# jepsen-io/maelstrom

Measured on NVIDIA H100. Metric: simulated msgs/sec (broadcast, 4096 nodes), higher is better.
Workload: dtype int64

## Files before the change

include/maelstrom_b200.h:

```cpp
#ifndef MAELSTROM_B200_H
#define MAELSTROM_B200_H

#include <stddef.h>
#include <stdint.h>

#ifdef __cplusplus
extern "C" {
#endif

#define MS_ABI_VERSION 2


typedef struct ms_msg {
  uint64_t id;
  int64_t  deadline_ns;
  uint32_t src, dest;
  uint32_t msg_id;
  uint32_t in_reply_to;
  uint16_t type;
  uint16_t flags;
  uint32_t p0;
  uint64_t p1;
} ms_msg;

// ... 141 lines not shown

typedef struct ms_kv_gen_config {
  uint32_t n_clients;
  uint32_t value_range;
  uint32_t keys_per_group;
  int64_t  interval_ns;
  int64_t  timeout_ns;
  int64_t  time_limit_ns;
  int64_t  key_period_ns;
} ms_kv_gen_config;
enum { MS_HF_KV_READ = 2, MS_HF_KV_WRITE = 3, MS_HF_KV_CAS = 4 };
int ms_add_kv_clients(ms_sim* sim, const ms_kv_gen_config* cfg, uint32_t first_name);

int ms_schedule_ops(ms_sim* sim, const ms_op* ops, size_t n);

int      ms_step(ms_sim* sim, uint64_t n_rounds);
int      ms_run(ms_sim* sim, int64_t until_virtual_ns);
int64_t  ms_now(ms_sim* sim);
uint64_t ms_round(ms_sim* sim);
int      ms_set_idle_jump(ms_sim* sim, int enable);

int ms_net_drop(ms_sim* sim, uint32_t src, uint32_t dest);
int ms_net_heal(ms_sim* sim);
int ms_net_slow(ms_sim* sim);
int ms_net_fast(ms_sim* sim);
int ms_net_flaky(ms_sim* sim);
int ms_net_set_loss(ms_sim* sim, double p);
int ms_net_partition(ms_sim* sim, const uint32_t* component_id, size_t n);

typedef struct ms_nemesis_config {
  uint32_t group;
  uint32_t targets;
  int64_t  interval_ns;
  int64_t  start_ns;
  int64_t  time_limit_ns;
} ms_nemesis_config;
#define MS_H_NEMESIS 0xFFFFFFFFu
enum { MS_HF_NEM_ONE = 5, MS_HF_NEM_MAJORITY = 6, MS_HF_NEM_MINORITY_THIRD = 7, MS_HF_NEM_STOP = 8,
       MS_HF_NEM_MAJORITIES_RING = 9 };
int ms_set_nemesis(ms_sim* sim, const ms_nemesis_config* cfg);
int ms_nemesis_grudge(uint32_t seed_lo, uint32_t seed_hi, uint32_t cluster, uint32_t g, uint32_t op, uint32_t target,
                      uint32_t* side_out);

int ms_journal_open(ms_sim* sim, const char* path);
int ms_journal_close(ms_sim* sim);
int ms_journal_drain(ms_sim* sim, ms_event* events, ms_jbody* bodies, size_t cap, size_t* n_out);
uint64_t ms_journal_written(ms_sim* sim);

enum { MS_JFMT_EVENT = 32, MS_JFMT_12 = 12, MS_JFMT_8 = 8, MS_JFMT_4 = 4,
       MS_JFMT_16 = 16 };
typedef struct ms_jround {
  uint64_t round;
  int64_t  time_ns;
  uint64_t ev_base;
  uint64_t id_ref;
} ms_jround;
typedef struct ms_jbatch {
  uint64_t first_event, n_events;
  uint64_t n_rounds;
  int64_t  now;
  uint64_t round, next_event;
  uint32_t format, overflow, more, error;
  uint64_t range_events;
} ms_jbatch;
typedef int (*ms_journal_sink)(void* ctx, const ms_jbatch* batch, const ms_jround* rounds, const void* events);
int ms_run_streamed(ms_sim* sim, int64_t until_virtual_ns, int format, size_t buf_events,
                    ms_journal_sink sink, void* ctx);
int ms_journal_decode(const ms_jbatch* batch, const ms_jround* rounds, const void* events, ms_event* out);
typedef struct ms_jdecoder ms_jdecoder;
ms_jdecoder* ms_jdecoder_create(uint32_t log2_window);
void ms_jdecoder_destroy(ms_jdecoder* dec);
int ms_jdecoder_decode(ms_jdecoder* dec, const ms_jbatch* batch, const ms_jround* rounds, const void* events, ms_event* out);
int ms_jdecoder_note(ms_jdecoder* dec, const ms_event* events, size_t n);
const char* ms_jdecoder_error(const ms_jdecoder* dec);

int ms_stats(ms_sim* sim, uint64_t out[9]);

size_t   ms_node_set(ms_sim* sim, uint32_t node, uint32_t* values, size_t cap);
uint64_t ms_client_replies(ms_sim* sim);
uint64_t ms_undeliverable(ms_sim* sim);
int      ms_raft_state(ms_sim* sim, uint32_t node, uint64_t out[8]);

int ms_counters(ms_sim* sim, uint64_t out[8]);

int ms_ring_counters(ms_sim* sim, uint64_t* out, uint32_t n);

int ms_set_origin(ms_sim* sim, uint64_t round, uint64_t msg_id, uint64_t event_id, uint32_t ring_pos,
                  uint32_t ring_stride);

#define MS_SHARD_BLOB_BYTES 512
typedef void (*ms_barrier_fn)(void* ctx, void* cuda_stream);
int   ms_shard_handles(ms_sim* sim, void* blob_out);
int   ms_shard_connect(ms_sim* sim, uint32_t peer, const void* blob);
int   ms_set_barrier(ms_sim* sim, ms_barrier_fn fn, void* ctx);
void* ms_stream(ms_sim* sim);
uint32_t ms_shard_owner(uint32_t e, uint32_t n_servers, uint32_t n_shards);

int ms_timer_begin(ms_sim* sim);
int ms_timer_end(ms_sim* sim, double* elapsed_ms);
int ms_profile(ms_sim* sim, int enable);
int ms_profile_read(ms_sim* sim, double* round_kernel_ms, uint64_t* launches);
int ms_debug_phase_cycles(ms_sim* sim, int enable, uint64_t out[64]);

size_t ms_topology(uint32_t topology, uint32_t n, uint32_t node, uint32_t* out, size_t cap);

#ifdef __cplusplus
}
#endif
#endif
```

integration/java/maelstrom/b200/Native.java:

```java
package maelstrom.b200;

import java.nio.ByteBuffer;

public final class Native {
  static { System.loadLibrary("ms_jni"); }
  private Native() {}

  public interface JournalSink { int accept(ByteBuffer batch, ByteBuffer rounds, ByteBuffer events); }

  public static native int abiVersion();
  public static native long create(ByteBuffer msConfig);
  public static native void destroy(long h);
  public static native String lastError(long h);
  public static native int startNodes(long h, int workload);
  public static native int stopNodes(long h);
  public static native int addEndpoint(long h, String id, int kind);
  public static native int removeEndpoint(long h, int idx);
  public static native int endpointIndex(long h, String id);
  public static native long send(long h, int src, int dest, int type, int flags, int msgId, int inReplyTo, int p0, long p1);
  public static native int recv(long h, int endpoint, long timeoutNs, ByteBuffer msMsg48);
  public static native long sendJson(long h, String line);
  public static native int recvJson(long h, int endpoint, long timeoutNs, ByteBuffer outUtf8, long cap);
  public static native int addGenClients(long h, ByteBuffer msGenConfig, int firstName);
  public static native int addKvClients(long h, ByteBuffer msKvGenConfig, int firstName);
  public static native long historyDrain(long h, ByteBuffer msHist32, long cap);
  public static native int scheduleOps(long h, ByteBuffer msOps, long n);
  public static native int step(long h, long nRounds);
  public static native int run(long h, long untilNs);
  public static native long now(long h);
  public static native long round(long h);
  public static native int setIdleJump(long h, int enable);
  public static native int netDrop(long h, int src, int dest);
  public static native int netHeal(long h);
  public static native int netSlow(long h);
  public static native int netFast(long h);
  public static native int netFlaky(long h);
  public static native int netSetLoss(long h, double p);
  public static native int netPartition(long h, ByteBuffer componentIds, long n);
  public static native int setNemesis(long h, ByteBuffer msNemesisConfig);
  public static native int nemesisGrudge(int seedLo, int seedHi, int cluster, int g, int op, int target, ByteBuffer sides);
  public static native int journalOpen(long h, String path);
  public static native int journalClose(long h);
  public static native long journalDrain(long h, ByteBuffer events, ByteBuffer bodies, long cap);
  public static native long journalWritten(long h);
  public static native int runStreamed(long h, long untilNs, int format, long bufEvents, JournalSink sink);
  public static native int journalDecode(ByteBuffer batch, ByteBuffer rounds, ByteBuffer events, ByteBuffer outEvents);
  public static native long jdecoderCreate(int log2Window);
  public static native void jdecoderDestroy(long decoder);
  public static native int jdecoderDecode(long decoder, ByteBuffer batch, ByteBuffer rounds, ByteBuffer events, ByteBuffer outEvents);
  public static native int jdecoderNote(long decoder, ByteBuffer events, long n);
  public static native String jdecoderError(long decoder);
  public static native int stats(long h, ByteBuffer out9);
  public static native long nodeSet(long h, int node, ByteBuffer values, long cap);
  public static native long clientReplies(long h);
  public static native long undeliverable(long h);
  public static native int raftState(long h, int node, ByteBuffer out8);
  public static native int counters(long h, ByteBuffer out8);
  public static native int ringCounters(long h, ByteBuffer out, int n);
  public static native int setOrigin(long h, long round, long msgId, long eventId, int ringPos, int ringStride);
  public static native int shardHandles(long h, ByteBuffer blob512);
  public static native int shardConnect(long h, int peer, ByteBuffer blob512);
  public static native int setBarrierDefault(long h);
  public static native long stream(long h);
  public static native int shardOwner(int endpoint, int nServers, int nShards);
  public static native int timerBegin(long h);
  public static native double timerEnd(long h);
  public static native int profile(long h, int enable);
  public static native int profileRead(long h, ByteBuffer out2);
  public static native int debugPhaseCycles(long h, int enable, ByteBuffer out64);
  public static native long topology(int topology, int n, int node, ByteBuffer out, long cap);
}
```

maelstrom_b200/_lib.py:

```python
import ctypes as C
import os

import numpy as np

_DIR = os.path.dirname(os.path.abspath(__file__))
SO_PATH = os.environ.get("MS_B200_LIB") or os.path.join(_DIR, "libmaelstrom_b200.so")

MSG_DTYPE = np.dtype([("id", "<u8"), ("deadline_ns", "<i8"), ("src", "<u4"), ("dest", "<u4"),
                      ("msg_id", "<u4"), ("in_reply_to", "<u4"), ("type", "<u2"), ("flags", "<u2"),
                      ("p0", "<u4"), ("p1", "<u8")])
EVENT_DTYPE = np.dtype([("event_id", "<u8"), ("time_ns", "<i8"), ("msg_id", "<u8"),
                        ("src", "<u4"), ("dest", "<u4")])
JBODY_DTYPE = np.dtype([("id", "<u8"), ("msg_id", "<u4"), ("in_reply_to", "<u4"), ("type", "<u2"),
                        ("flags", "<u2"), ("p0", "<u4"), ("p1", "<u8")])
BODY_DTYPE = np.dtype([("type", "<u2"), ("flags", "<u2"), ("msg_id", "<u4"), ("in_reply_to", "<u4"),
                       ("p0", "<u4"), ("p1", "<u8")])
OP_DTYPE = np.dtype([("time_ns", "<i8"), ("src", "<u4"), ("dest", "<u4"), ("body", BODY_DTYPE)])
assert MSG_DTYPE.itemsize == 48 and EVENT_DTYPE.itemsize == 32 and JBODY_DTYPE.itemsize == 32
assert BODY_DTYPE.itemsize == 24 and OP_DTYPE.itemsize == 40


class Config(C.Structure):
    _fields_ = [("n_nodes", C.c_uint32), ("workload", C.c_uint32), ("topology", C.c_uint32),
                ("latency_dist", C.c_uint32), ("latency_mean_ms", C.c_uint32),
# ... 15 lines not shown

class GenConfig(C.Structure):
    _fields_ = [("n_clients", C.c_uint32), ("read_permille", C.c_uint32), ("interval_ns", C.c_int64),
                ("timeout_ns", C.c_int64), ("time_limit_ns", C.c_int64), ("quiet_ns", C.c_int64)]


class KvGenConfig(C.Structure):
    _fields_ = [("n_clients", C.c_uint32), ("value_range", C.c_uint32), ("keys_per_group", C.c_uint32),
                ("interval_ns", C.c_int64), ("timeout_ns", C.c_int64), ("time_limit_ns", C.c_int64),
                ("key_period_ns", C.c_int64)]


class NemesisConfig(C.Structure):
    _fields_ = [("group", C.c_uint32), ("targets", C.c_uint32), ("interval_ns", C.c_int64), ("start_ns", C.c_int64),
                ("time_limit_ns", C.c_int64)]


HIST_DTYPE = np.dtype([("time_ns", "<i8"), ("order", "<u8"), ("client", "<u4"), ("op", "<u4"), ("type", "u1"),
                       ("f", "u1"), ("error", "<u2"), ("value", "<u4")])
assert HIST_DTYPE.itemsize == 32


class JBatch(C.Structure):
    _fields_ = [("first_event", C.c_uint64), ("n_events", C.c_uint64), ("n_rounds", C.c_uint64),
                ("now", C.c_int64), ("round", C.c_uint64), ("next_event", C.c_uint64),
                ("format", C.c_uint32), ("overflow", C.c_uint32), ("more", C.c_uint32), ("error", C.c_uint32),
                ("range_events", C.c_uint64)]


JROUND_DTYPE = np.dtype([("round", "<u8"), ("time_ns", "<i8"), ("ev_base", "<u8"), ("id_ref", "<u8")])
JOURNAL_SINK = C.CFUNCTYPE(C.c_int, C.c_void_p, C.POINTER(JBatch), C.c_void_p, C.c_void_p)
JFMT_EVENT, JFMT_12, JFMT_8, JFMT_16, JFMT_4 = 32, 12, 8, 16, 4

_P = C.c_void_p
SYMBOLS = {
    "ms_abi_version": (C.c_uint32, []),
    "ms_create": (_P, [C.POINTER(Config)]),
    "ms_destroy": (None, [_P]),
    "ms_last_error": (C.c_char_p, [_P]),
    "ms_start_nodes": (C.c_int, [_P, C.c_uint32]),
    "ms_stop_nodes": (C.c_int, [_P]),
    "ms_add_endpoint": (C.c_int, [_P, C.c_char_p, C.c_int]),
    "ms_remove_endpoint": (C.c_int, [_P, C.c_uint32]),
    "ms_endpoint_index": (C.c_int, [_P, C.c_char_p]),
    "ms_send": (C.c_int64, [_P, C.c_uint32, C.c_uint32, C.POINTER(Body)]),
    "ms_recv": (C.c_int, [_P, C.c_uint32, C.c_int64, _P]),
    "ms_send_json": (C.c_int64, [_P, C.c_char_p]),
    "ms_recv_json": (C.c_int, [_P, C.c_uint32, C.c_int64, C.c_char_p, C.c_size_t]),
    "ms_add_gen_clients": (C.c_int, [_P, _P, C.c_uint32]),
    "ms_add_kv_clients": (C.c_int, [_P, _P, C.c_uint32]),
    "ms_history_drain": (C.c_int, [_P, _P, C.c_size_t, C.POINTER(C.c_size_t)]),
    "ms_schedule_ops": (C.c_int, [_P, _P, C.c_size_t]),
    "ms_step": (C.c_int, [_P, C.c_uint64]),
    "ms_run": (C.c_int, [_P, C.c_int64]),
    "ms_now": (C.c_int64, [_P]),
    "ms_round": (C.c_uint64, [_P]),
    "ms_set_idle_jump": (C.c_int, [_P, C.c_int]),
    "ms_net_drop": (C.c_int, [_P, C.c_uint32, C.c_uint32]),
    "ms_net_heal": (C.c_int, [_P]),
    "ms_net_slow": (C.c_int, [_P]),
    "ms_net_fast": (C.c_int, [_P]),
    "ms_net_flaky": (C.c_int, [_P]),
    "ms_net_set_loss": (C.c_int, [_P, C.c_double]),
    "ms_net_partition": (C.c_int, [_P, _P, C.c_size_t]),
    "ms_set_nemesis": (C.c_int, [_P, _P]),
    "ms_nemesis_grudge": (C.c_int, [C.c_uint32, C.c_uint32, C.c_uint32, C.c_uint32, C.c_uint32, C.c_uint32, _P]),
    "ms_journal_open": (C.c_int, [_P, C.c_char_p]),
    "ms_journal_close": (C.c_int, [_P]),
    "ms_journal_drain": (C.c_int, [_P, _P, _P, C.c_size_t, C.POINTER(C.c_size_t)]),
    "ms_journal_written": (C.c_uint64, [_P]),
    "ms_run_streamed": (C.c_int, [_P, C.c_int64, C.c_int, C.c_size_t, JOURNAL_SINK, _P]),
    "ms_journal_decode": (C.c_int, [C.POINTER(JBatch), _P, _P, _P]),
    "ms_jdecoder_create": (_P, [C.c_uint32]),
    "ms_jdecoder_destroy": (None, [_P]),
    "ms_jdecoder_decode": (C.c_int, [_P, C.POINTER(JBatch), _P, _P, _P]),
    "ms_jdecoder_note": (C.c_int, [_P, _P, C.c_size_t]),
    "ms_jdecoder_error": (C.c_char_p, [_P]),
    "ms_stats": (C.c_int, [_P, _P]),
    "ms_node_set": (C.c_size_t, [_P, C.c_uint32, _P, C.c_size_t]),
    "ms_client_replies": (C.c_uint64, [_P]),
    "ms_undeliverable": (C.c_uint64, [_P]),
    "ms_raft_state": (C.c_int, [_P, C.c_uint32, _P]),
    "ms_counters": (C.c_int, [_P, _P]),
    "ms_ring_counters": (C.c_int, [_P, _P, C.c_uint32]),
    "ms_set_origin": (C.c_int, [_P, C.c_uint64, C.c_uint64, C.c_uint64, C.c_uint32, C.c_uint32]),
    "ms_timer_begin": (C.c_int, [_P]),
    "ms_timer_end": (C.c_int, [_P, C.POINTER(C.c_double)]),
    "ms_profile": (C.c_int, [_P, C.c_int]),
    "ms_profile_read": (C.c_int, [_P, C.POINTER(C.c_double), C.POINTER(C.c_uint64)]),
    "ms_shard_handles": (C.c_int, [_P, _P]),
    "ms_shard_connect": (C.c_int, [_P, C.c_uint32, _P]),
    "ms_set_barrier": (C.c_int, [_P, _P, _P]),
    "ms_stream": (_P, [_P]),
    "ms_shard_owner": (C.c_uint32, [C.c_uint32, C.c_uint32, C.c_uint32]),
    "ms_debug_phase_cycles": (C.c_int, [_P, C.c_int, _P]),
    "ms_topology": (C.c_size_t, [C.c_uint32, C.c_uint32, C.c_uint32, _P, C.c_size_t]),
}

SHARD_BLOB_BYTES = 512
BARRIER_FN = C.CFUNCTYPE(None, C.c_void_p, C.c_void_p)
_lib = None


def lib():
    global _lib
    if _lib is None:
        if not os.path.exists(SO_PATH):
            raise ImportError(
                "maelstrom_b200: %s is missing -- run `python -c 'import __graft_entry__ as g; g.build()'` "
                "(nvcc, sm_90a). There is no CPU fallback." % SO_PATH)
        L = C.CDLL(SO_PATH)
        for name, (res, args) in SYMBOLS.items():
            fn = getattr(L, name)
            fn.restype = res
            fn.argtypes = args
        _lib = L
    return _lib
```

maelstrom_b200/csrc/ms_device.cuh:

```cuda
#pragma once
#include <stdint.h>
#include "../../include/maelstrom_b200.h"

#if defined(__CUDACC__)
#define MS_HD __host__ __device__ __forceinline__
#else
#define MS_HD inline
#endif

namespace msd {

constexpr int64_t  kTickNs   = 1000000;
constexpr uint32_t kInjector = 0xFFFFFFFFu;
constexpr uint8_t  kRemoved  = 0x80;

enum : uint32_t {
  E_NONE = 0, E_RING_OVERFLOW = 1, E_WINDOW_OVERFLOW = 2, E_JOURNAL_OVERFLOW = 3,
  E_INVALID_DEST = 4, E_HISTORY = 5, E_VALUE_RANGE = 6, E_MAIL_OVERFLOW = 7,
  E_CALENDAR_OVERFLOW = 8, E_ID_RANGE = 9, E_BARRIER = 10, E_SNAPSHOT = 11,
  E_RAFT_CAPACITY = 12, E_HISTORY_RING = 13
};

#ifndef MS_CLS0_NT
#define MS_CLS0_NT 64
#endif
#ifndef MS_CLS1_NT
#define MS_CLS1_NT 128
#endif
constexpr int kClsThreads[4] = {MS_CLS0_NT, MS_CLS1_NT, 256, 512};
constexpr uint32_t kClsLadder[4] = {128u, 512u, 2048u, 32768u};

struct DevState {
  int64_t  now;
  int64_t  stop_ns;
  uint64_t round;
  uint64_t next_id;
  uint64_t next_event;
  uint64_t journal_drained;
  uint64_t drain_round;
  uint64_t jraw_cursor;
  uint64_t jraw_drained;
  uint64_t stats[6];
  uint64_t lost;
  uint64_t part_drops;
  uint64_t client_replies;
  uint64_t rounds_run;
  uint64_t fallback_sorts;
  uint64_t undeliverable;
  uint64_t gc_hist_n;
  uint64_t gc_hist_drained;
  uint32_t done;
  uint32_t zero_pending;
  uint32_t error;
  uint32_t error_arg;
  uint32_t inj_count;
  uint32_t sched_cursor;
  uint32_t mail_count;
  uint32_t time_advanced;
  uint32_t max_window_seen;
  uint32_t cal_release;
  uint32_t cal_free_n;
  uint32_t cal_ret_n;
  uint32_t slot_open;
  uint32_t bar_epoch;
  uint32_t cls_count[2][4];
  uint32_t cls_small[2][4];
  uint32_t cls_cursor[2][4];
  uint64_t idle_wake;
  int64_t  nem_next;
};

struct RoundMeta {
  uint64_t round;
  int64_t  now;
  uint64_t id_base;
  uint64_t ev_base;
  uint64_t raw_base;
  uint32_t n_tickets;
  uint32_t pad;
  uint64_t ev_total, em_total;
};

struct NetParams {
  uint64_t loss_thresh;
  uint64_t exp_coeff;
  uint32_t dist;
  uint32_t mean_ms;
  uint32_t scale;
  uint32_t pair_active;
  uint32_t comp_active;
  uint32_t any_removed;
};

struct Params {
  DevState* st;
  NetParams* np;
  uint8_t*  kind;
  uint32_t* tail;
  uint32_t* limit;
  uint32_t* head;
  uint64_t* ep_born;
  uint4*    ring;
  uint32_t  ring_cap, ring_cap_s;
  uint32_t  n_ep, n_servers, n_inj_tickets, max_window, max_window_s;
  size_t    cring_off;
  uint32_t  cq;
  RoundMeta* rmeta;
  uint32_t* rt_em;
  uint32_t* rt_ev;
  uint64_t* rt_chunk;
  uint64_t* rt_cnt;
  uint64_t* phase_cycles;
  uint32_t  n_shards, shard_id;
  uint4*    ring_sh[8];
  uint32_t* tail_sh[8];
  uint32_t* head_sh[8];
  uint64_t* rt_cnt_sh[8];
  uint32_t* bar_sh[8];
  uint32_t  hist, hist_mask, t_max, n_classes;
  uint32_t  split_commit;
  uint32_t  n_sms;
  uint64_t* cm_blk;
  uint32_t* cm_flags;
  uint32_t* cls_list;
  uint32_t  cls_cap[4];
  uint4*    jraw;
  uint4*    jbody;
  uint64_t  jmask;
  uint32_t  jlevel, jdiscard;
  uint32_t* pair_bits;
  uint32_t  pair_words;
  uint32_t* comp;
  uint32_t  seed_lo, seed_hi;
  uint32_t  workload, topology, n_values, bm_words;
  uint32_t* bitmap;
  uint32_t* nbr_off;
  uint32_t* nbr;
  uint32_t* next_msg_id;
  uint32_t* set_count;
  ms_msg*   inj_buf;
  const ms_op* sched;
  uint32_t  n_sched;
  const uint32_t* tick_off;
  uint32_t  n_tick_off;
  ms_msg*   mail;
  uint32_t  mail_cap;
  uint4*    cal;
  uint32_t* cal_count;
  uint32_t* cal_tab;
  uint32_t* cal_par;
  uint32_t* cal_free;
  uint32_t* cal_ret;
// ... 184 lines not shown
```

maelstrom_b200/csrc/ms_engine.cu:

```cuda
#include <cuda_runtime.h>
#include <math.h>
#include <stdio.h>
#include <stdlib.h>
#include <string.h>

#include <algorithm>
#include <deque>
#include <mutex>
#include <new>
#include <string>
#include <unordered_map>
#include <vector>

#include "ms_device.cuh"
#include "ms_nemesis.h"
#include "ms_tree.h"
#include "ms_fressian.h"
#include "ms_json.h"

using namespace msd;

extern "C" {
cudaError_t msk_round_smem_attr(size_t bytes);
size_t msk_round_smem_bytes(uint32_t cap);
// ... 307 lines not shown
      }
    }
    launch_rounds_direct(n, jump);
  }

  void launch_rounds_direct(uint64_t n, bool jump = false) {
    const bool glue = P.n_shards > 1 && !use_calendar && !barrier && !P.cm_blk && P.n_ep <= 32768 && !getenv("MS_NO_GLUE");
    for (uint64_t i = 0; i < n; i++) {
      cudaEvent_t a = nullptr, b = nullptr;
      if (profiling) {
        if (prof_used + 2 > prof_ev.size()) {
          prof_ev.resize(prof_used + 2, nullptr);
          cudaEventCreate(&prof_ev[prof_used]);
          cudaEventCreate(&prof_ev[prof_used + 1]);
        }
        a = prof_ev[prof_used]; b = prof_ev[prof_used + 1];
        prof_used += 2;
      }
      const int T = (int)(P.n_inj_tickets + P.n_ep);
      int grids[4];
      for (int c = 0; c < n_classes; c++) grids[c] = std::max(1, std::min(class_grid[c], T));
      if (P.n_shards <= 1) {
        if (jump) {
          msk_launch_idle_jump(&P, stream);
          if (!capturing()) launches += 2;
        }
        if (P.nem) {
          msk_launch_nemesis(&P, stream);
          if (!capturing()) launches += 1;
        }
        msk_launch_round(&P, n_classes, class_cap, class_threads, grids, use_calendar ? 1 : 0, stream, a, b, 15, aux_streams, aux_events);
        if (!capturing()) launches += (use_calendar ? 2 : 1) + n_classes + (P.split_commit ? (P.cm_blk ? 3 : 1) : 0);
      } else if (glue) {
        msk_launch_round(&P, n_classes, class_cap, class_threads, grids, 0, stream, a, b, 16, aux_streams, aux_events);
        msk_launch_round(&P, n_classes, class_cap, class_threads, grids, 0, stream, a, b, 2, aux_streams, aux_events);
        if (!capturing()) launches += 1 + n_classes;
      } else {
        if (use_calendar) {
          msk_launch_round(&P, n_classes, class_cap, class_threads, grids, 1, stream, a, b, 1, aux_streams, aux_events);
          do_barrier();
        }
        msk_launch_round(&P, n_classes, class_cap, class_threads, grids, 0, stream, a, b, 8, aux_streams, aux_events);
        do_barrier();
        msk_launch_round(&P, n_classes, class_cap, class_threads, grids, 0, stream, a, b, 2, aux_streams, aux_events);
        do_barrier();
        msk_launch_round(&P, n_classes, class_cap, class_threads, grids, 0, stream, a, b, 4, aux_streams, aux_events);
        if (!capturing()) launches += (use_calendar ? 2 : 1) + n_classes + (use_calendar ? 4 : 3);
      }
    }
    if (glue && n) {
      int grids[4] = {1, 1, 1, 1};
      msk_launch_round(&P, n_classes, class_cap, class_threads, grids, 0, stream, nullptr, nullptr, 32, aux_streams, aux_events);
      if (!capturing()) launches += 1;
    }
  }

  bool capturing() {
    cudaStreamCaptureStatus st_ = cudaStreamCaptureStatusNone;
    cudaStreamIsCapturing(stream, &st_);
    return st_ != cudaStreamCaptureStatusNone;
  }

  void collect_profile() {
    for (size_t i = 0; i + 1 < prof_used; i += 2) {
      float ms = 0;
      if (cudaEventElapsedTime(&ms, prof_ev[i], prof_ev[i + 1]) == cudaSuccess) { prof_ms += ms; prof_launches++; }
    }
    prof_used = 0;
  }

  int maybe_flush_journal_file() {
    if (!jfile || cfg.journal_discard || cfg.journal_level == 0) return MS_OK;
    if (hs.jraw_cursor - hs.jraw_drained < (P.jmask + 1) / 4 && hs.round - hs.drain_round < P.hist / 4) return MS_OK;
    return flush_journal_file();
  }

  int drain(ms_event* ev, ms_jbody* bodies, size_t cap, size_t* n_out) {
    *n_out = 0;
    if (cfg.journal_level == 0 || cfg.journal_discard) return MS_OK;
    const uint64_t avail = hs.next_event - hs.journal_drained;
    const size_t n = (size_t)std::min<uint64_t>(avail, cap);
    if (n == 0) return MS_OK;
    if (!stage_ev) {
      stage_cap = (size_t)std::min<uint64_t>(P.jmask + 1, 1ull << 22);
      CK(cudaMalloc(&stage_ev, stage_cap * 32));
      if (cfg.journal_level >= 2) CK(cudaMalloc(&stage_body, stage_cap * 32));
    }
    hmeta.resize(P.hist);
    CK(cudaMemcpy(hmeta.data(), P.rmeta, (size_t)P.hist * sizeof(RoundMeta), cudaMemcpyDeviceToHost));
    auto meta = [&](uint64_t r) -> const RoundMeta& { return hmeta[(size_t)(r & P.hist_mask)]; };
    size_t done = 0;
    while (done < n) {
      const size_t piece = std::min(n - done, stage_cap);
      const uint64_t first = hs.journal_drained;
      const uint64_t r0 = hs.drain_round;
      uint64_t r1 = r0;
      while (r1 < hs.round && meta(r1).round == r1 && meta(r1).ev_base < first + piece) r1++;
      if (r1 == r0) { set_err("journal drain: round history lost"); return MS_ERR_SIM; }
      const bool want_body = bodies && cfg.journal_level >= 2;
      if (P.n_shards > 1) {
        CK(cudaMemsetAsync(stage_ev, 0xFF, piece * 32, stream));
        if (want_body) CK(cudaMemsetAsync(stage_body, 0xFF, piece * 32, stream));
      }
      msk_journal_expand(&P, r0, (uint32_t)(r1 - r0), first, piece, stage_ev, want_body ? stage_body : nullptr, n_sms, stream);
      CK(cudaStreamSynchronize(stream));
      CK(cudaMemcpy(ev + done, stage_ev, piece * 32, cudaMemcpyDeviceToHost));
      if (want_body) CK(cudaMemcpy(bodies + done, stage_body, piece * 32, cudaMemcpyDeviceToHost));
      done += piece;
      hs.journal_drained += piece;
      while (hs.drain_round < hs.round && meta(hs.drain_round).ev_base + meta(hs.drain_round).ev_total <= hs.journal_drained)
        hs.drain_round++;
    }
    hs.jraw_drained = hs.drain_round < hs.round ? meta(hs.drain_round).raw_base : hs.jraw_cursor;
    CK(cudaMemcpy(&P.st->journal_drained, &hs.journal_drained, sizeof(uint64_t), cudaMemcpyHostToDevice));
    CK(cudaMemcpy(&P.st->drain_round, &hs.drain_round, sizeof(uint64_t), cudaMemcpyHostToDevice));
    CK(cudaMemcpy(&P.st->jraw_drained, &hs.jraw_drained, sizeof(uint64_t), cudaMemcpyHostToDevice));
    *n_out = n;
    return MS_OK;
  }

  int flush_journal_file() {
    if (!jfile) return MS_OK;
    std::vector<ms_event> ev(1 << 16);
    std::vector<ms_jbody> bd(cfg.journal_level >= 2 ? (1 << 16) : 0);
    for (;;) {
      size_t n = 0;
      const int rc = drain(ev.data(), bd.empty() ? nullptr : bd.data(), ev.size(), &n);
      if (rc) return rc;
      if (!n) break;
      for (size_t i = 0; i < n; i++) {
        if (jfress) { write_fressian_event(ev[i], bd[i]); continue; }
        fwrite(&ev[i], sizeof(ms_event), 1, jfile);
        if (!bd.empty()) fwrite(&bd[i], sizeof(ms_jbody), 1, jfile);
      }
    }
    fflush(jfile);
    return MS_OK;
  }

  void write_fressian_event(const ms_event& e, const ms_jbody& b) {
    const std::string tname = type_name(b.type);
    std::vector<msf::Writer::KV> kv;
    kv.push_back({"type", true, 0, tname});
    if (b.flags & MS_F_MSG_ID) kv.push_back({"msg_id", false, (int64_t)b.msg_id, ""});
    if (b.flags & MS_F_REPLY) kv.push_back({"in_reply_to", false, (int64_t)b.in_reply_to, ""});
    const bool kv_peer = (e.src < kinds.size() && (kinds[e.src] & 0x7F) == MS_KIND_SERVICE) ||
                         (e.dest < kinds.size() && (kinds[e.dest] & 0x7F) == MS_KIND_SERVICE) || cfg.workload == MS_W_RAFT;
    const int64_t lo = (int64_t)(b.p1 & 0xFFFFFFFFull), hi = (int64_t)(b.p1 >> 32);
    switch (b.type) {
      case MS_T_BROADCAST: kv.push_back({"message", false, (int64_t)b.p0, ""}); break;
      case MS_T_ADD: case MS_T_REPLICATE_ONE: kv.push_back({"element", false, (int64_t)b.p0, ""}); break;
      case MS_T_ERROR: kv.push_back({"code", false, (int64_t)b.p0, ""}); break;
      case MS_T_ECHO: case MS_T_ECHO_OK: kv.push_back({"echo_handle", false, (int64_t)b.p1, ""}); break;
      case MS_T_READ: if (kv_peer) kv.push_back({"key", false, (int64_t)b.p0, ""}); break;
      case MS_T_READ_OK:
        if (kv_peer) kv.push_back({"value", false, (int64_t)b.p1, ""});
        else kv.push_back({"count", false, (int64_t)b.p0, ""});
        break;
      case MS_T_WRITE: kv.push_back({"key", false, (int64_t)b.p0, ""}); kv.push_back({"value", false, lo, ""}); break;
      case MS_T_CAS:
        kv.push_back({"key", false, (int64_t)b.p0, ""}); kv.push_back({"from", false, lo, ""}); kv.push_back({"to", false, hi, ""});
        break;
      case MS_T_TS_OK: kv.push_back({"ts", false, (int64_t)b.p1, ""}); break;
      case MS_T_REPLICATE_FULL: kv.push_back({"count", false, (int64_t)b.p0, ""}); kv.push_back({"snapshot", false, (int64_t)b.p1, ""}); break;
      case MS_T_REQUEST_VOTE:
        kv.push_back({"term", false, (int64_t)b.p0, ""}); kv.push_back({"last_log_index", false, lo, ""});
        kv.push_back({"last_log_term", false, hi, ""});
// ... 102 lines not shown
  }
  {
    const uint32_t* ladder = kClsLadder;
    const int thr_gset[4] = {256, 256, 256, 512};
    const int* thr = c.workload == MS_W_GSET ? thr_gset : kClsThreads;
    s->n_classes = 0;
    for (int k = 0; k < 4; k++) {
      const uint32_t cap = std::min(ladder[k], c.max_window);
      s->class_cap[s->n_classes] = cap;
      s->class_threads[s->n_classes] = c.threads_per_node ? (int)c.threads_per_node : thr[k];
      s->n_classes++;
      if (cap == c.max_window) break;
    }
  }

  int ndev = 0;
  if (cudaGetDeviceCount(&ndev) != cudaSuccess || ndev == 0) {
    set_err("no CUDA device: maelstrom_b200 has no CPU fallback");
    return MS_ERR_CUDA;
  }
  s->device = c.device;
  CK(cudaSetDevice(s->device));
  CK(cudaStreamCreateWithFlags(&s->stream, cudaStreamNonBlocking));
  for (int k = 0; k < 4; k++) CK(cudaStreamCreateWithFlags(&s->aux_streams[k], cudaStreamNonBlocking));
  for (int k = 0; k < 5; k++) CK(cudaEventCreateWithFlags(&s->aux_events[k], cudaEventDisableTiming));

  Params& P = s->P;
  memset(&P, 0, sizeof P);
  const uint32_t M = c.max_endpoints;
  const bool compact = c.workload == MS_W_BROADCAST;
  const size_t n_ctr = (size_t)M + (compact ? c.n_nodes : 0u);
  int rc;
  if ((rc = s->dalloc(&P.st, 1))) return rc;
  if ((rc = s->dalloc(&P.np, 1))) return rc;
  if ((rc = s->dalloc(&P.kind, M))) return rc;
  if ((rc = s->dalloc(&P.tail, n_ctr))) return rc;
  if ((rc = s->dalloc(&P.limit, n_ctr))) return rc;
  if ((rc = s->dalloc(&P.head, n_ctr))) return rc;
  if ((rc = s->dalloc(&P.ep_born, M))) return rc;
  {
    const size_t full_vecs = ((size_t)c.n_nodes * c.server_ring_cap + (size_t)(M - c.n_nodes) * c.ring_cap) * 3;
    const size_t compact_vecs = compact ? (size_t)c.n_nodes * c.server_ring_cap : 0;
    void* ptr = nullptr;
    CK(cudaMalloc(&ptr, (full_vecs + compact_vecs) * 16));
    s->allocs.push_back(ptr);
    P.ring = (uint4*)ptr;
    P.cring_off = full_vecs;
    P.cq = compact ? M : 0u;
  }
  P.ring_cap = c.ring_cap;
  P.ring_cap_s = c.server_ring_cap;
  P.n_servers = c.n_nodes;
  P.n_ep = c.n_nodes;
  P.n_inj_tickets = 8;
  P.max_window = c.max_window;
  P.max_window_s = c.server_max_window;
  s->use_graph = c.reserved[1] == 1;
  P.n_shards = c.n_shards;
  P.shard_id = c.shard_id;
  {
    P.t_max = M + P.n_inj_tickets;
    const uint32_t hist = history_rows(c.reserved[0], P.t_max);
    P.hist = hist;
    P.hist_mask = hist - 1;
    if ((rc = s->dalloc(&P.rmeta, hist))) return rc;
    if ((rc = s->dalloc(&P.rt_em, (size_t)hist * P.t_max))) return rc;
    if ((rc = s->dalloc(&P.rt_ev, (size_t)hist * P.t_max))) return rc;
    if ((rc = s->dalloc(&P.rt_chunk, (size_t)hist * P.t_max))) return rc;
    if ((rc = s->dalloc(&P.rt_cnt, (size_t)hist * P.t_max))) return rc;
    std::vector<RoundMeta> init(hist);
    memset(init.data(), 0, init.size() * sizeof(RoundMeta));
    for (uint32_t i = 1; i < hist; i++) init[i].round = ~0ull;
    CK(cudaMemcpyAsync(P.rmeta, init.data(), init.size() * sizeof(RoundMeta), cudaMemcpyHostToDevice, s->stream));
    CK(cudaStreamSynchronize(s->stream));
  }
  P.jlevel = c.journal_level;
  P.jdiscard = c.journal_discard;
  if (c.journal_level) {
    const uint64_t J = 1ull << c.journal_cap_log2;
    void* ptr = nullptr;
    CK(cudaMalloc(&ptr, J * 16));
    s->allocs.push_back(ptr);
    P.jraw = (uint4*)ptr;
    P.jmask = J - 1;
    if (c.journal_level >= 2) {
      CK(cudaMalloc(&ptr, J * 32));
      s->allocs.push_back(ptr);
      P.jbody = (uint4*)ptr;
    }
  }
  if ((rc = s->dalloc(&P.comp, M))) return rc;
  P.seed_lo = c.seed_lo;
  P.seed_hi = c.seed_hi;
  P.workload = c.workload;
  P.topology = c.topology;
  P.n_values = c.n_values;
  P.bm_words = (c.n_values + 31) / 32;
  if (c.workload == MS_W_BROADCAST || c.workload == MS_W_GSET) {
    if ((rc = s->dalloc(&P.bitmap, (size_t)c.n_nodes * P.bm_words))) return rc;
    if ((rc = s->dalloc(&P.set_count, c.n_nodes))) return rc;
    if (c.topology != MS_TOPO_TOTAL) {
      std::vector<uint32_t> off(c.n_nodes + 1, 0), nbr, tmp;
      for (uint32_t k = 0; k < c.n_nodes; k++) {
        topo_neighbors(c.topology, c.n_nodes, k, tmp);
        nbr.insert(nbr.end(), tmp.begin(), tmp.end());
        off[k + 1] = (uint32_t)nbr.size();
      }
      if ((rc = s->dalloc(&P.nbr_off, off.size()))) return rc;
      if ((rc = s->dalloc(&P.nbr, nbr.size() + 1))) return rc;
      CK(cudaMemcpyAsync(P.nbr_off, off.data(), off.size() * 4, cudaMemcpyHostToDevice, s->stream));
      if (!nbr.empty()) CK(cudaMemcpyAsync(P.nbr, nbr.data(), nbr.size() * 4, cudaMemcpyHostToDevice, s->stream));
      CK(cudaStreamSynchronize(s->stream));
    }
  } else if (c.workload == MS_W_ECHO) {
    if ((rc = s->dalloc(&P.next_msg_id, c.n_nodes))) return rc;
  }
  P.family = c.workload == MS_W_GSET ? 1u : (c.workload >= MS_W_RAFT ? 4u : 0u);
  if (c.workload == MS_W_TXN_TREE) {
    if (c.n_shards > 1) { set_err("MS_W_TXN_TREE runs on one GPU (tree records are read across nodes)"); return MS_ERR_ARG; }
    const size_t N = c.n_nodes;
    P.tt_per_node = c.reserved[3] ? c.reserved[3] : 256u;
    P.tt_cache_mask = pow2_at_least(c.reserved[4] ? c.reserved[4] : 1024u) - 1u;
    const uint64_t n_ptrs = 2ull + (uint64_t)N * P.tt_per_node;
    if (n_ptrs > (1ull << 31)) { set_err("MS_W_TXN_TREE: n_nodes x reserved[3] pointers do not fit"); return MS_ERR_ARG; }
    if (!c.reserved[2]) c.reserved[2] = (uint32_t)n_ptrs;
    if ((rc = s->dalloc(&P.tt_node, N)) || (rc = s->dalloc(&P.tt_recs, (size_t)n_ptrs * 64)) ||
        (rc = s->dalloc(&P.tt_cache, N * ((size_t)P.tt_cache_mask + 1))) || (rc = s->dalloc(&P.tt_queue, N * kTreeQueue)))
      return rc;
    mst::Rec empty{};
    empty.type = 1; empty.lo = 0; empty.hi = (uint8_t)mst::kRing; empty.n = 0;
    CK(cudaMemcpyAsync(P.tt_recs + (size_t)(mst::kPtrEmpty - 1u) * 64, &empty, sizeof empty, cudaMemcpyHostToDevice, s->stream));
    CK(cudaStreamSynchronize(s->stream));
  }
  if (c.workload == MS_W_TXN || c.workload == MS_W_TXN_TREE) {
    const size_t N = c.n_nodes;
    P.rf_stage_cap = c.workload == MS_W_TXN_TREE ? c.server_max_window * (mst::kMaxWrites + 2u) + 64u : c.server_max_window + 16u;
    P.rf_cb_mask = pow2_at_least(c.reserved[5] ? c.reserved[5] : kRaftCallbacks) - 1u;
    if (c.workload == MS_W_TXN_TREE && P.rf_cb_mask + 1u < 128u) P.rf_cb_mask = 127u;
    if ((rc = s->dalloc(&P.rf_node, N)) || (rc = s->dalloc(&P.rf_cb, N * ((size_t)P.rf_cb_mask + 1) * 2)) ||
        (rc = s->dalloc(&P.rf_stage, N * P.rf_stage_cap * 3)))
      return rc;
  }
  if (c.workload == MS_W_RAFT) {
    const size_t N = c.n_nodes;
    P.rf_n_keys = c.reserved[2] ? c.reserved[2] : 4096u;
    P.rf_log_cap = c.reserved[3] ? c.reserved[3] : 4096u;
    P.rf_group = (c.reserved[4] && c.reserved[4] < c.n_nodes) ? c.reserved[4] : 0u;
    P.rf_gmax = P.rf_group ? P.rf_group : c.n_nodes;
    P.rf_cb_mask = pow2_at_least(c.reserved[5] ? c.reserved[5] : kRaftCallbacks) - 1u;
    P.rf_stage_cap = c.server_max_window + 2u * P.rf_gmax + P.rf_log_cap + 16u;
    P.rf_vote_words = (P.rf_gmax + 31u) / 32u;
    const uint64_t heap_want = std::max<uint64_t>(std::max<uint64_t>(1u << 16, 8ull * P.rf_log_cap), 64ull * c.n_nodes);
    if (heap_want > (1ull << 30)) { set_err("Raft payload heap too large"); return MS_ERR_ARG; }
    const uint32_t heap_words = pow2_at_least((uint32_t)heap_want);
    P.rf_heap_mask = heap_words - 1u;
    if ((rc = s->dalloc(&P.rf_node, N)) || (rc = s->dalloc(&P.rf_log, N * P.rf_log_cap * 2)) ||
        (rc = s->dalloc(&P.rf_kv_val, N * P.rf_n_keys)) || (rc = s->dalloc(&P.rf_kv_has, N * P.rf_n_keys)) ||
        (rc = s->dalloc(&P.rf_next, N * P.rf_gmax)) || (rc = s->dalloc(&P.rf_match, N * P.rf_gmax)) ||
        (rc = s->dalloc(&P.rf_scratch, N * P.rf_gmax)) || (rc = s->dalloc(&P.rf_cb, N * ((size_t)P.rf_cb_mask + 1) * 2)) ||
        (rc = s->dalloc(&P.rf_votes, N * P.rf_vote_words)) || (rc = s->dalloc(&P.rf_stage, N * P.rf_stage_cap * 3)) ||
        (rc = s->dalloc(&P.rf_heap, (size_t)heap_words)) || (rc = s->dalloc(&P.rf_heap_cursor, 1)) ||
        (rc = s->dalloc(&P.rf_ext_off, N * kRaftExt + (N * kRaftExt + 1) / 2)))
      return rc;
    P.rf_ext_tag = reinterpret_cast<uint32_t*>(P.rf_ext_off + N * kRaftExt);
    P.rf_heap_sh[c.shard_id] = P.rf_heap;
    P.rf_ext_off_sh[c.shard_id] = P.rf_ext_off;
    P.rf_ext_tag_sh[c.shard_id] = P.rf_ext_tag;
// ... 1093 lines not shown

int ms_jdecoder_decode(ms_jdecoder* d, const ms_jbatch* b, const ms_jround* rounds, const void* events, ms_event* out) {
  if (!d || !b || !rounds || !events || !out) return MS_ERR_ARG;
  if (b->n_events && !b->n_rounds) { d->err = "ms_jdecoder: batch without round rows"; return MS_ERR_ARG; }
  if (b->format != MS_JFMT_4) {
    const int rc = ms_journal_decode(b, rounds, events, out);
    return rc ? rc : ms_jdecoder_note(d, out, (size_t)b->n_events);
  }
  const uint32_t* w = (const uint32_t*)events;
  size_t r = 0;
  for (uint64_t k = 0; k < b->n_events; k++) {
    const uint64_t g = b->first_event + k;
    while (r + 1 < b->n_rounds && rounds[r + 1].ev_base <= g) r++;
    if (g == rounds[r].ev_base) {
      d->next_send = rounds[r].id_ref;
    } else if (k == 0 && (!d->have || d->expect_event != g)) {
      d->err = "ms_jdecoder: batch starts inside a round the decoder has not followed (event " + std::to_string(g) + ")";
      return MS_ERR_ARG;
    }
    ms_event e;
    e.time_ns = rounds[r].time_ns;
    if (w[k] & 0x80000000u) {
      const uint64_t id = rounds[r].id_ref - 1ull - (uint64_t)(w[k] & 0x7FFFFFFFu);
      if (d->tag[id & d->mask] != id + 1) {
        d->err = "ms_jdecoder: the :send of message " + std::to_string(id) + " is not in the decoder's window";
        return MS_ERR_ARG;
      }
      const uint64_t sd = d->sd[id & d->mask];
      e.event_id = g | MS_EVENT_RECV; e.msg_id = id; e.src = (uint32_t)sd; e.dest = (uint32_t)(sd >> 32);
    } else {
      const uint64_t id = d->next_send++;
      e.event_id = g; e.msg_id = id; e.src = (w[k] >> 16) & 0x7FFFu; e.dest = w[k] & 0xFFFFu;
      d->tag[id & d->mask] = id + 1;
      d->sd[id & d->mask] = (uint64_t)e.src | ((uint64_t)e.dest << 32);
    }
    out[k] = e;
  }
  d->expect_event = b->first_event + b->n_events;
  d->have = true;
  return MS_OK;
}

int ms_stats(ms_sim* s, uint64_t out[9]) {
  std::lock_guard<std::mutex> g(s->mu);
  const uint64_t snd[3] = {s->hs.stats[2] + s->hs.stats[4], s->hs.stats[2], s->hs.stats[4]};
  const uint64_t rcv[3] = {s->hs.stats[3] + s->hs.stats[5], s->hs.stats[3], s->hs.stats[5]};
  for (int c = 0; c < 3; c++) {
    out[c * 3 + 0] = snd[c];
    out[c * 3 + 1] = rcv[c];
    out[c * 3 + 2] = snd[c];
  }
  return MS_OK;
}

size_t ms_node_set(ms_sim* s, uint32_t node, uint32_t* values, size_t cap) {
  std::lock_guard<std::mutex> g(s->mu);
  cudaSetDevice(s->device);
  if (node >= s->cfg.n_nodes || !s->P.bitmap) return 0;
  std::vector<uint32_t> w(s->P.bm_words);
  if (cudaMemcpy(w.data(), s->P.bitmap + (size_t)node * s->P.bm_words, w.size() * 4, cudaMemcpyDeviceToHost) != cudaSuccess)
    return 0;
  size_t n = 0;
  for (uint32_t i = 0; i < s->P.bm_words; i++)
    for (uint32_t b = 0; b < 32; b++)
      if ((w[i] >> b) & 1u) { if (values && n < cap) values[n] = i * 32 + b; n++; }
  return n;
}

uint64_t ms_client_replies(ms_sim* s) { std::lock_guard<std::mutex> g(s->mu); return s->hs.client_replies; }
uint64_t ms_undeliverable(ms_sim* s) { std::lock_guard<std::mutex> g(s->mu); return s->hs.undeliverable; }

int ms_raft_state(ms_sim* s, uint32_t node, uint64_t out[8]) {
  std::lock_guard<std::mutex> g(s->mu);
  cudaSetDevice(s->device);
  if (!s->P.rf_node || node >= s->cfg.n_nodes) { set_err("ms_raft_state: not a Raft node"); return MS_ERR_ARG; }
  RaftDev r;
  CK(cudaStreamSynchronize(s->stream));
  CK(cudaMemcpy(&r, s->P.rf_node + node, sizeof r, cudaMemcpyDeviceToHost));
  out[0] = (uint64_t)r.state; out[1] = r.term; out[2] = (uint64_t)(r.voted_for + 1); out[3] = r.commit_index;
  out[4] = r.last_applied; out[5] = (uint64_t)(r.leader + 1); out[6] = r.log_size; out[7] = r.kv_size;
  return MS_OK;
}

int ms_counters(ms_sim* s, uint64_t out[8]) {
  std::lock_guard<std::mutex> g(s->mu);
  out[0] = s->hs.rounds_run;
  out[1] = s->hs.stats[2] + s->hs.stats[4];
  out[2] = s->hs.stats[3] + s->hs.stats[5];
  out[3] = s->launches;
  out[4] = s->hs.lost;
  out[5] = s->hs.part_drops;
  out[6] = s->hs.max_window_seen;
  out[7] = s->hs.fallback_sorts;
  return MS_OK;
}

int ms_ring_counters(ms_sim* s, uint64_t* out, uint32_t n) {
  std::lock_guard<std::mutex> g(s->mu);
  cudaSetDevice(s->device);
  const uint32_t S = s->P.n_servers;
  if (!out || n < 6u * S) { set_err("ms_ring_counters: out needs 6 x n_nodes entries"); return MS_ERR_ARG; }
  std::vector<uint32_t> t(S), l(S), h(S);
  memset(out, 0, (size_t)6 * S * sizeof(uint64_t));
  CK(cudaStreamSynchronize(s->stream));
  for (uint32_t part = 0; part < 2; part++) {
    if (part == 1 && !s->P.cq) break;
    const size_t off = part ? s->P.cq : 0u;
    CK(cudaMemcpy(t.data(), s->P.tail + off, S * 4, cudaMemcpyDeviceToHost));
    CK(cudaMemcpy(l.data(), s->P.limit + off, S * 4, cudaMemcpyDeviceToHost));
    CK(cudaMemcpy(h.data(), s->P.head + off, S * 4, cudaMemcpyDeviceToHost));
    uint64_t* o = out + (size_t)part * 3 * S;
    for (uint32_t e = 0; e < S; e++) {
      if (owner_of(e, S, s->P.n_shards) != s->P.shard_id) continue;
      o[e] = t[e]; o[S + e] = l[e]; o[2 * S + e] = h[e];
    }
  }
  return (int)S;
}

int ms_set_origin(ms_sim* s, uint64_t round, uint64_t msg_id, uint64_t event_id, uint32_t ring_pos, uint32_t ring_stride) {
  std::lock_guard<std::mutex> g(s->mu);
  cudaSetDevice(s->device);
  if (round >= (1ull << 39) || msg_id >= (1ull << 62) || event_id >= (1ull << 62)) {
    set_err("ms_set_origin: round must be < 2^39 (order keys), msg_id and event_id < 2^62");
    return MS_ERR_ARG;
  }
  if (s->hs.rounds_run || !s->pending.empty() || !s->sched.empty()) {
    set_err("ms_set_origin: only a fresh simulation (no send, schedule or round yet) can be moved");
    return MS_ERR_ARG;
  }
  Params& P = s->P;
  CK(cudaStreamSynchronize(s->stream));
  s->hs.round = round;
  s->hs.drain_round = round;
  s->hs.next_id = msg_id;
  s->hs.next_event = event_id;
  s->hs.journal_drained = event_id;
  CK(cudaMemcpy(P.st, &s->hs, sizeof(DevState), cudaMemcpyHostToDevice));
  std::vector<RoundMeta> rows(P.hist);
  memset(rows.data(), 0, rows.size() * sizeof(RoundMeta));
  for (RoundMeta& m : rows) m.round = ~0ull;
  RoundMeta& r0 = rows[(size_t)(round & P.hist_mask)];
  r0.round = round;
  r0.now = s->hs.now;
  r0.id_base = msg_id;
  r0.ev_base = event_id;
  r0.raw_base = s->hs.jraw_cursor;
  CK(cudaMemcpy(P.rmeta, rows.data(), rows.size() * sizeof(RoundMeta), cudaMemcpyHostToDevice));
  const uint32_t M = s->cfg.max_endpoints;
  std::vector<uint64_t> born(M, msg_id);
  CK(cudaMemcpy(P.ep_born, born.data(), (size_t)M * 8, cudaMemcpyHostToDevice));
  const size_t n_ctr = (size_t)M + (P.cq ? P.n_servers : 0u);
  std::vector<uint32_t> ctr(n_ctr);
  CK(cudaMemcpy(ctr.data(), P.tail, n_ctr * 4, cudaMemcpyDeviceToHost));
  for (size_t i = 0; i < n_ctr; i++) {
    const uint32_t e = i < M ? (uint32_t)i : (uint32_t)(i - P.cq);
    if (owner_of(e, P.n_servers, P.n_shards) == P.shard_id) ctr[i] = ring_pos + e * ring_stride;
  }
  CK(cudaMemcpy(P.tail, ctr.data(), n_ctr * 4, cudaMemcpyHostToDevice));
  CK(cudaMemcpy(P.limit, ctr.data(), n_ctr * 4, cudaMemcpyHostToDevice));
  CK(cudaMemcpy(P.head, ctr.data(), n_ctr * 4, cudaMemcpyHostToDevice));
  return MS_OK;
}

int ms_set_idle_jump(ms_sim* s, int enable) {
  std::lock_guard<std::mutex> g(s->mu);
  if (enable && s->P.n_shards > 1) { set_err("ms_set_idle_jump: a sharded simulation ticks (the jump would need the minimum over all shards)"); return MS_ERR_ARG; }
  if (enable && s->cfg.reserved[1] == 1) { set_err("ms_set_idle_jump: not with CUDA-graph replay (ms_config.reserved[1] = 1)"); return MS_ERR_ARG; }
  s->idle_jump = enable != 0;
  return MS_OK;
}

struct ShardBlob {
  uint32_t magic, shard_id, n_shards, t_max;
  uint32_t max_endpoints, ring_cap, hist, pad;
  cudaIpcMemHandle_t ring, tail, head, rt_cnt, bar;
// ... 162 lines not shown
```

maelstrom_b200/csrc/ms_jni.c:

```c
#if defined(__has_include)
#if __has_include(<jni.h>)
#define MS_HAVE_JNI 1
#endif
#endif

#ifdef MS_HAVE_JNI
#include <jni.h>
#include <stdint.h>
#include <string.h>
#include "maelstrom_b200.h"

#define H(h) ((ms_sim*)(intptr_t)(h))
#define FN(name) JNIEXPORT JNICALL Java_maelstrom_b200_Native_##name
#define BUF(b) ((b) ? (*env)->GetDirectBufferAddress(env, (b)) : NULL)

jint FN(abiVersion)(JNIEnv* env, jclass c) { (void)env; (void)c; return (jint)ms_abi_version(); }

jlong FN(create)(JNIEnv* env, jclass c, jobject cfg) {
  (void)c;
  return (jlong)(intptr_t)ms_create((const ms_config*)BUF(cfg));
}
void FN(destroy)(JNIEnv* env, jclass c, jlong h) { (void)env; (void)c; ms_destroy(H(h)); }
jstring FN(lastError)(JNIEnv* env, jclass c, jlong h) { (void)c; return (*env)->NewStringUTF(env, ms_last_error(H(h))); }

// ... 67 lines not shown
jint FN(netDrop)(JNIEnv* env, jclass c, jlong h, jint src, jint dest) { (void)env; (void)c; return ms_net_drop(H(h), (uint32_t)src, (uint32_t)dest); }
jint FN(netHeal)(JNIEnv* env, jclass c, jlong h) { (void)env; (void)c; return ms_net_heal(H(h)); }
jint FN(netSlow)(JNIEnv* env, jclass c, jlong h) { (void)env; (void)c; return ms_net_slow(H(h)); }
jint FN(netFast)(JNIEnv* env, jclass c, jlong h) { (void)env; (void)c; return ms_net_fast(H(h)); }
jint FN(netFlaky)(JNIEnv* env, jclass c, jlong h) { (void)env; (void)c; return ms_net_flaky(H(h)); }
jint FN(netSetLoss)(JNIEnv* env, jclass c, jlong h, jdouble p) { (void)env; (void)c; return ms_net_set_loss(H(h), p); }
jint FN(netPartition)(JNIEnv* env, jclass c, jlong h, jobject comp, jlong n) {
  (void)c;
  return ms_net_partition(H(h), (const uint32_t*)BUF(comp), (size_t)n);
}
jint FN(setNemesis)(JNIEnv* env, jclass c, jlong h, jobject cfg) {
  (void)c;
  return ms_set_nemesis(H(h), (const ms_nemesis_config*)BUF(cfg));
}
jint FN(nemesisGrudge)(JNIEnv* env, jclass c, jint seedLo, jint seedHi, jint cluster, jint g, jint op, jint target,
                       jobject sides) {
  (void)c;
  return ms_nemesis_grudge((uint32_t)seedLo, (uint32_t)seedHi, (uint32_t)cluster, (uint32_t)g, (uint32_t)op,
                           (uint32_t)target, (uint32_t*)BUF(sides));
}

jint FN(journalOpen)(JNIEnv* env, jclass c, jlong h, jstring path) {
  (void)c;
  const char* s = (*env)->GetStringUTFChars(env, path, 0);
  const int rc = ms_journal_open(H(h), s);
  (*env)->ReleaseStringUTFChars(env, path, s);
  return rc;
}
jint FN(journalClose)(JNIEnv* env, jclass c, jlong h) { (void)env; (void)c; return ms_journal_close(H(h)); }
jlong FN(journalDrain)(JNIEnv* env, jclass c, jlong h, jobject events, jobject bodies, jlong cap) {
  (void)c;
  size_t n = 0;
  const int rc = ms_journal_drain(H(h), (ms_event*)BUF(events), (ms_jbody*)BUF(bodies), (size_t)cap, &n);
  return rc < 0 ? (jlong)rc : (jlong)n;
}
jlong FN(journalWritten)(JNIEnv* env, jclass c, jlong h) { (void)env; (void)c; return (jlong)ms_journal_written(H(h)); }

struct ms_jni_sink { JNIEnv* env; jobject sink; jmethodID accept; };
static int ms_jni_sink_call(void* ctx, const ms_jbatch* b, const ms_jround* rounds, const void* events) {
  struct ms_jni_sink* k = (struct ms_jni_sink*)ctx;
  JNIEnv* env = k->env;
  jobject jb = (*env)->NewDirectByteBuffer(env, (void*)b, (jlong)sizeof *b);
  jobject jr = (*env)->NewDirectByteBuffer(env, (void*)rounds, (jlong)(b->n_rounds * sizeof *rounds));
  jobject je = (*env)->NewDirectByteBuffer(env, (void*)events, (jlong)(b->n_events * b->format));
  const jint rc = (*env)->CallIntMethod(env, k->sink, k->accept, jb, jr, je);
  (*env)->DeleteLocalRef(env, jb); (*env)->DeleteLocalRef(env, jr); (*env)->DeleteLocalRef(env, je);
  return (*env)->ExceptionCheck(env) ? 1 : (int)rc;
}
jint FN(runStreamed)(JNIEnv* env, jclass c, jlong h, jlong untilNs, jint format, jlong bufEvents, jobject sink) {
  (void)c;
  struct ms_jni_sink k;
  k.env = env; k.sink = sink;
  k.accept = (*env)->GetMethodID(env, (*env)->GetObjectClass(env, sink), "accept",
                                 "(Ljava/nio/ByteBuffer;Ljava/nio/ByteBuffer;Ljava/nio/ByteBuffer;)I");
  if (!k.accept) return MS_ERR_ARG;
  return ms_run_streamed(H(h), untilNs, format, (size_t)bufEvents, ms_jni_sink_call, &k);
}
jint FN(journalDecode)(JNIEnv* env, jclass c, jobject batch, jobject rounds, jobject events, jobject out) {
  (void)c;
  return ms_journal_decode((const ms_jbatch*)BUF(batch), (const ms_jround*)BUF(rounds), BUF(events), (ms_event*)BUF(out));
}
jlong FN(jdecoderCreate)(JNIEnv* env, jclass c, jint log2Window) { (void)env; (void)c; return (jlong)(intptr_t)ms_jdecoder_create((uint32_t)log2Window); }
void FN(jdecoderDestroy)(JNIEnv* env, jclass c, jlong d) { (void)env; (void)c; ms_jdecoder_destroy((ms_jdecoder*)(intptr_t)d); }
jint FN(jdecoderDecode)(JNIEnv* env, jclass c, jlong d, jobject batch, jobject rounds, jobject events, jobject out) {
  (void)c;
  return ms_jdecoder_decode((ms_jdecoder*)(intptr_t)d, (const ms_jbatch*)BUF(batch), (const ms_jround*)BUF(rounds), BUF(events),
                            (ms_event*)BUF(out));
}
jint FN(jdecoderNote)(JNIEnv* env, jclass c, jlong d, jobject events, jlong n) {
  (void)c;
  return ms_jdecoder_note((ms_jdecoder*)(intptr_t)d, (const ms_event*)BUF(events), (size_t)n);
}
jstring FN(jdecoderError)(JNIEnv* env, jclass c, jlong d) { (void)c; return (*env)->NewStringUTF(env, ms_jdecoder_error((const ms_jdecoder*)(intptr_t)d)); }

jint FN(stats)(JNIEnv* env, jclass c, jlong h, jobject out9) { (void)c; return ms_stats(H(h), (uint64_t*)BUF(out9)); }
jlong FN(nodeSet)(JNIEnv* env, jclass c, jlong h, jint node, jobject values, jlong cap) {
  (void)c;
  return (jlong)ms_node_set(H(h), (uint32_t)node, (uint32_t*)BUF(values), (size_t)cap);
}
jlong FN(clientReplies)(JNIEnv* env, jclass c, jlong h) { (void)env; (void)c; return (jlong)ms_client_replies(H(h)); }
jlong FN(undeliverable)(JNIEnv* env, jclass c, jlong h) { (void)env; (void)c; return (jlong)ms_undeliverable(H(h)); }
jint FN(raftState)(JNIEnv* env, jclass c, jlong h, jint node, jobject out8) { (void)c; return ms_raft_state(H(h), (uint32_t)node, (uint64_t*)BUF(out8)); }
jint FN(counters)(JNIEnv* env, jclass c, jlong h, jobject out8) { (void)c; return ms_counters(H(h), (uint64_t*)BUF(out8)); }
jint FN(ringCounters)(JNIEnv* env, jclass c, jlong h, jobject out, jint n) { (void)c; return ms_ring_counters(H(h), (uint64_t*)BUF(out), (uint32_t)n); }
jint FN(setOrigin)(JNIEnv* env, jclass c, jlong h, jlong round, jlong msg_id, jlong event_id, jint ring_pos, jint ring_stride) {
  (void)env; (void)c;
  return ms_set_origin(H(h), (uint64_t)round, (uint64_t)msg_id, (uint64_t)event_id, (uint32_t)ring_pos, (uint32_t)ring_stride);
}

jint FN(shardHandles)(JNIEnv* env, jclass c, jlong h, jobject blob) { (void)c; return ms_shard_handles(H(h), BUF(blob)); }
jint FN(shardConnect)(JNIEnv* env, jclass c, jlong h, jint peer, jobject blob) { (void)c; return ms_shard_connect(H(h), (uint32_t)peer, BUF(blob)); }
jint FN(setBarrierDefault)(JNIEnv* env, jclass c, jlong h) { (void)env; (void)c; return ms_set_barrier(H(h), NULL, NULL); }
jlong FN(stream)(JNIEnv* env, jclass c, jlong h) { (void)env; (void)c; return (jlong)(intptr_t)ms_stream(H(h)); }
jint FN(shardOwner)(JNIEnv* env, jclass c, jint e, jint nServers, jint nShards) {
  (void)env; (void)c;
  return (jint)ms_shard_owner((uint32_t)e, (uint32_t)nServers, (uint32_t)nShards);
}

jint FN(timerBegin)(JNIEnv* env, jclass c, jlong h) { (void)env; (void)c; return ms_timer_begin(H(h)); }
jdouble FN(timerEnd)(JNIEnv* env, jclass c, jlong h) {
  (void)env; (void)c;
  double ms = 0;
  return ms_timer_end(H(h), &ms) < 0 ? -1.0 : ms;
}
jint FN(profile)(JNIEnv* env, jclass c, jlong h, jint enable) { (void)env; (void)c; return ms_profile(H(h), enable); }
jint FN(profileRead)(JNIEnv* env, jclass c, jlong h, jobject out2) {
  (void)c;
  unsigned char* o = (unsigned char*)BUF(out2);
  double ms = 0; uint64_t n = 0;
  const int rc = ms_profile_read(H(h), &ms, &n);
  memcpy(o, &ms, 8); memcpy(o + 8, &n, 8);
  return rc;
}
jint FN(debugPhaseCycles)(JNIEnv* env, jclass c, jlong h, jint enable, jobject out64) { (void)c; return ms_debug_phase_cycles(H(h), enable, (uint64_t*)BUF(out64)); }
jlong FN(topology)(JNIEnv* env, jclass c, jint topo, jint n, jint node, jobject out, jlong cap) {
  (void)c;
  return (jlong)ms_topology((uint32_t)topo, (uint32_t)n, (uint32_t)node, (uint32_t*)BUF(out), (size_t)cap);
}
#else
typedef int ms_jni_translation_unit_is_empty_without_a_jdk;
#endif
```

maelstrom_b200/csrc/ms_kernels.cu:

```cuda
#include <cuda_runtime.h>
#include <stdint.h>
#include "ms_device.cuh"
#include "ms_nemesis.h"

namespace msd {

#define FULL 0xFFFFFFFFu
#ifndef MS_EMUL
#define MS_LAUNCH(kern, grid, block, smem, stream, ...) kern<<<(grid), (block), (smem), (stream)>>>(__VA_ARGS__)
#endif
constexpr int MAXB = 64;
constexpr int MAXNB = 8;
constexpr uint64_t RECV_BIT = 1ull << 63;
constexpr uint32_t kResolvedTicket = 0xFFFFFFu;

__device__ __forceinline__ void st_v4(uint4* p, uint4 v) {
#ifdef MS_EMUL
  *p = v;
#else
  asm volatile("st.global.L1::no_allocate.v4.u32 [%0], {%1,%2,%3,%4};" ::"l"(p), "r"(v.x), "r"(v.y),
               "r"(v.z), "r"(v.w)
               : "memory");
#endif
}
// ... 111 lines not shown
  if (m->round != round || ticket >= p.t_max) {
    latch_error(st, E_HISTORY, (uint32_t)round);
    return 0;
  }
  return m->id_base + p.rt_em[(size_t)row * p.t_max + ticket];
}

__device__ __forceinline__ uint64_t cta_excl_scan_u64(uint64_t sum, int nt, int lane, int warp, uint64_t* wtmp ) {
  uint64_t incl = sum;
#pragma unroll
  for (int d = 1; d < 32; d <<= 1) {
    const uint64_t y = __shfl_up_sync(FULL, incl, d);
    if (lane >= d) incl += y;
  }
  if (lane == 31) wtmp[warp] = incl;
  __syncthreads();
  if (warp == 0) {
    const int nw = nt >> 5;
    const uint64_t w = lane < nw ? wtmp[lane] : 0;
    uint64_t wi = w;
#pragma unroll
    for (int d = 1; d < 32; d <<= 1) {
      const uint64_t y = __shfl_up_sync(FULL, wi, d);
      if (lane >= d) wi += y;
    }
    wtmp[lane] = wi - w;
    if (lane == 31) wtmp[32] = wi;
  }
  __syncthreads();
  return wtmp[warp] + incl - sum;
}

__device__ uint64_t block_excl_scan(uint64_t* a, int n, uint64_t* wtmp ) {
  const int nt = blockDim.x, tid = threadIdx.x, lane = tid & 31, warp = tid >> 5;
  const int c = (n + nt - 1) / nt;
  const int lo = min(tid * c, n), hi = min(lo + c, n);
  uint64_t sum = 0;
  for (int i = lo; i < hi; i++) sum += a[i];
  uint64_t run = cta_excl_scan_u64(sum, nt, lane, warp, wtmp);
  for (int i = lo; i < hi; i++) {
    const uint64_t v = a[i];
    a[i] = run;
    run += v;
  }
  const uint64_t total = wtmp[32];
  if (tid == 0) a[n] = total;
  __syncthreads();
  return total;
}

__device__ void block_bitonic_sort_idx(uint16_t* ord, const uint64_t* keyA, const uint32_t* keyB, int np) {
  const int nt = blockDim.x, tid = threadIdx.x;
  for (int k = 2; k <= np; k <<= 1) {
    for (int j = k >> 1; j > 0; j >>= 1) {
      for (int t = tid; t < (np >> 1); t += nt) {
        const int i = ((t & ~(j - 1)) << 1) | (t & (j - 1));
        const int l = i | j;
        const bool asc = (i & k) == 0;
        const uint16_t a = ord[i], b = ord[l];
        bool gt;
        if (a == 0xFFFF) gt = (b != 0xFFFF);
        else if (b == 0xFFFF) gt = false;
        else gt = keyA[a] > keyA[b] || (keyA[a] == keyA[b] && keyB[a] > keyB[b]);
        if (gt == asc) { ord[i] = b; ord[l] = a; }
      }
      __syncthreads();
    }
  }
}

struct EmitCtx {
  int64_t now;
  uint64_t round;
  uint64_t chunk;
  uint32_t n_recv;
  uint32_t ticket;
  uint32_t emitter;
  uint32_t idx_bias;
  bool need_rng;
  uint64_t const_lat;
  uint32_t c_send_cl, c_send_sv, c_lost, c_zero;
};

__device__ __forceinline__ void journal_raw(const Params& p, uint64_t pos, uint64_t id_or_idx, bool recv,
                                            const Rec& r) {
  if (p.jlevel == 0) return;
  const uint64_t v = id_or_idx | (recv ? RECV_BIT : 0ull);
  st_v4(p.jraw + (pos & p.jmask), make_uint4((uint32_t)v, (uint32_t)(v >> 32), r.src, r.dest));
  if (p.jlevel >= 2) {
    uint4* b = p.jbody + (pos & p.jmask) * 2;
    st_v4(b + 0, make_uint4((uint32_t)v, (uint32_t)(v >> 32), r.msg_id, r.in_reply_to));
    st_v4(b + 1, make_uint4(r.tf, r.p0, (uint32_t)r.p1, (uint32_t)(r.p1 >> 32)));
  }
}

__device__ __forceinline__ void journal_claim(const Params& p, DevState* st, uint32_t n, uint32_t ticket, uint64_t& chunk) {
  chunk = (n && p.jlevel) ? atomicAdd((unsigned long long*)&st->jraw_cursor, (unsigned long long)n) : 0ull;
  if (n && p.jlevel && !p.jdiscard && chunk + n - st->jraw_drained > p.jmask + 1)
    latch_error(st, E_JOURNAL_OVERFLOW, ticket);
}

__device__ __forceinline__ uint32_t ld_volatile_u32(const uint32_t* p) {
#ifdef MS_EMUL
  return __atomic_load_n(p, __ATOMIC_RELAXED);
#else
  return *reinterpret_cast<const volatile uint32_t*>(p);
#endif
}

__device__ uint32_t wheel_block(const Params& p, DevState* st, uint32_t* entry, bool designated) {
  uint32_t b = ld_volatile_u32(entry);
  if (b) return b - 1;
  if (!designated) {
    for (int spin = 0; spin < 64; spin++) {
      __nanosleep(64);
      b = ld_volatile_u32(entry);
      if (b) return b - 1;
    }
  }
  const uint32_t n = atomicAdd(&st->cal_free_n, 0xFFFFFFFFu);
  if (n == 0 || n > p.cal_blocks) {
    atomicAdd(&st->cal_free_n, 1u);
    latch_error(st, E_CALENDAR_OVERFLOW, 0xFFFFFFFFu);
    return 0xFFFFFFFFu;
  }
  const uint32_t mine = p.cal_free[n - 1];
  const uint32_t old = atomicCAS(entry, 0u, mine + 1u);
  if (old == 0u) return mine;
  p.cal_ret[atomicAdd(&st->cal_ret_n, 1u)] = mine;
  return old - 1u;
}

__device__ __forceinline__ void wheel_file(const Params& p, DevState* st, bool valid, uint32_t slot, const Rec& r) {
  const int lane = threadIdx.x & 31;
  const uint32_t key = valid ? slot : (0x80000000u | (uint32_t)lane);
  const uint32_t mask = __match_any_sync(FULL, key);
  const int leader = __ffs(mask) - 1;
  const uint32_t rank = __popc(mask & ((1u << lane) - 1u));
  uint32_t gen = 0, base = 0;
  if (valid && lane == leader) {
    gen = p.cal_par[slot];
    base = atomicAdd(&p.cal_count[(size_t)gen * p.cal_slots + slot], (uint32_t)__popc(mask));
  }
  gen = __shfl_sync(FULL, gen, leader);
  base = __shfl_sync(FULL, base, leader);
  if (!valid) return;
  const uint32_t k = base + rank;
  const uint32_t j = k >> p.cal_blk_log2, off = k & ((1u << p.cal_blk_log2) - 1u);
  if (j >= p.cal_tab_cap) { latch_error(st, E_CALENDAR_OVERFLOW, slot); return; }
  const uint32_t b = wheel_block(p, st, p.cal_tab + ((size_t)gen * p.cal_slots + slot) * p.cal_tab_cap + j, off == 0);
  if (b == 0xFFFFFFFFu) return;
  rec_store(p.cal + (((size_t)b << p.cal_blk_log2) + off) * 3, r);
}

__device__ __forceinline__ void emit_one(const Params& p, DevState* st, const NetParams& np, EmitCtx& cx,
                                         bool valid, Rec& r, uint32_t local_idx, uint32_t direct_pos,
                                         bool has_direct) {
  const int lane = threadIdx.x & 31;
  bool push = false, wheel = false;
  uint32_t wslot = 0;
  const bool undeliverable = valid && (r.dest >= p.n_ep || r.src >= p.n_ep ||
                                       (np.any_removed && ((p.kind[r.dest] | p.kind[r.src]) & kRemoved)));
  if (valid) {
    r.round = cx.round; r.ticket = cx.ticket; r.idx = local_idx;
    uint32_t x[4] = {0xFFFFFFFFu, 0, 0, 0};
    if (cx.need_rng)
      philox4x32_10(local_idx + cx.idx_bias, cx.emitter, (uint32_t)cx.round, (uint32_t)(cx.round >> 32),
                    p.seed_lo, p.seed_hi, x);
    const bool cl = (r.src >= p.n_servers && r.src < p.n_ep && kind_is_client(p.kind[r.src])) ||
                    (r.dest >= p.n_servers && r.dest < p.n_ep && kind_is_client(p.kind[r.dest]));
    const uint64_t lat = cl ? 0ull : (cx.need_rng ? latency_ms(np, x) : cx.const_lat);
    journal_raw(p, cx.chunk + cx.n_recv + local_idx, local_idx, false, r);
    if (cl) cx.c_send_cl++; else cx.c_send_sv++;
    if (undeliverable) {
      atomicAdd((unsigned long long*)&st->undeliverable, 1ull);
    } else if ((uint64_t)x[0] < np.loss_thresh) {
      cx.c_lost++;
    } else if (lat == 0) {
      cx.c_zero++;
      if (has_direct) {
        uint4* ring_o = p.ring_sh[owner_of(r.dest, p.n_servers, p.n_shards)];
        rec_store(ring_slot(p, ring_o, r.dest, direct_pos), r);
      } else {
        push = true;
      }
    } else {
      const uint64_t tick = (uint64_t)(cx.now / kTickNs) + lat;
      const uint64_t laps = (lat - 1) / p.cal_slots;
      if (p.cal == nullptr || laps > 0xFFFFu) {
        latch_error(st, E_CALENDAR_OVERFLOW, (uint32_t)lat);
      } else {
        wheel = true;
        wslot = (uint32_t)tick & (p.cal_slots - 1);
        r.round |= laps << 48;
      }
    }
  }
  if (__any_sync(FULL, wheel)) wheel_file(p, st, wheel, wslot, r);
  if (!__any_sync(FULL, push)) return;
  const uint32_t key = push ? r.dest : (0x80000000u | (uint32_t)lane);
  const uint32_t mask = __match_any_sync(FULL, key);
  const int leader = __ffs(mask) - 1;
  const uint32_t rank = __popc(mask & ((1u << lane) - 1u));
  uint32_t base = 0;
  const uint32_t o = push ? owner_of(r.dest, p.n_servers, p.n_shards) : 0u;
  if (push && lane == leader) base = atomicAdd(&p.tail_sh[o][r.dest], (uint32_t)__popc(mask));
  base = __shfl_sync(FULL, base, leader);
  if (push) {
    const uint32_t pos = base + rank;
    if ((uint32_t)(pos - p.head_sh[o][r.dest]) >= ring_cap_of(p, r.dest)) {
      latch_error(st, E_RING_OVERFLOW, r.dest);
    } else {
      rec_store(ring_slot(p, p.ring_sh[o], r.dest, pos), r);
    }
  }
}

__global__ void k_set_bit(uint32_t* words, size_t word, uint32_t bit) { atomicOr(words + word, 1u << bit); }

__device__ __forceinline__ void gen_hist(const Params& p, DevState* st, int64_t now, uint64_t round, uint32_t e,
                                         const GenDev& g, uint32_t op, uint32_t type, uint32_t f, uint32_t error, uint32_t value) {
  const unsigned long long pos = atomicAdd((unsigned long long*)&st->gc_hist_n, 1ull);
  if (pos - st->gc_hist_drained > p.gc_hist_mask) { latch_error(st, E_HISTORY_RING, e); return; }
  uint4* at = p.gc_hist + (pos & p.gc_hist_mask) * 2;
  const uint64_t order = (round << 24) | g.ordinal;
  at[0] = make_uint4((uint32_t)now, (uint32_t)((uint64_t)now >> 32), (uint32_t)order, (uint32_t)(order >> 32));
  at[1] = make_uint4(e, op, type | (f << 8) | (error << 16), value);
}

__device__ __forceinline__ bool gen_timer_due(const Params& p, const GenDev& g, int64_t now) {
  if (g.waiting_for) return now >= g.deadline_ns;
  if (g.phase == GEN_MIX) return now >= p.gc_limit_ns || now >= g.next_op_ns;
  if (g.phase == GEN_QUIET) return now >= p.gc_limit_ns + p.gc_quiet_ns;
  return g.phase == GEN_FINAL;
}
__device__ __forceinline__ int64_t gen_wake_ns(const Params& p, const GenDev& g) {
  if (g.waiting_for) return g.deadline_ns;
  if (g.phase == GEN_MIX) return min(p.gc_limit_ns, g.next_op_ns);
  if (g.phase == GEN_QUIET) return p.gc_limit_ns + p.gc_quiet_ns;
  return g.phase == GEN_FINAL ? INT64_MIN : INT64_MAX;
}

__device__ bool gen_step(const Params& p, DevState* st, uint32_t e, int64_t now, uint64_t round, const uint4* myring,
                         uint32_t head, uint32_t my_mask, uint32_t n, const uint16_t* ord, const uint32_t* vals, Rec& out) {
  GenDev g = p.gc[e];
  for (uint32_t pos = 0; pos < n; pos++) {
    const uint32_t i = ord[pos];
    if (!(vals[i] & (1u << 30))) continue;
    const uint4* rp = myring + (size_t)((head + i) & my_mask) * 3;
    const uint4 vb = rp[1], vc = rp[2];
    const uint32_t type = vc.x & 0xFFFFu, flags = vc.x >> 16;
    if (!g.waiting_for || !(flags & MS_F_REPLY) || vb.w != g.waiting_for) continue;
    uint32_t outcome = MS_H_OK, err = 0, value = g.cur_value;
    if (type == MS_T_ERROR) {
      err = vc.y;
// ... 1036 lines not shown
    uint32_t ck = 0xFFFFFFFFu, cval = 0;
    bool chas = false, cdirty = false;
    for (uint32_t pos = 0; pos < n && svc < 4; pos++) {
      const uint32_t i = sm.ord[pos];
      if (!(sm.vals[i] & V_RECV)) continue;
      SvReq q;
      q.type = sm.meta[i] & 0xFFu; q.flags = sm.meta[i] >> 8; q.key = skey[pos];
      q.p1 = sm.reg1[pos];
      q.src = 0;
      if (svc == MS_SVC_SEQ_KV)
        q.src = (w.ring + (size_t)((w.head + i) & w.mask) * 3)[1].x;
      const bool keyed = q.type == MS_T_READ || q.type == MS_T_WRITE || q.type == MS_T_CAS;
      if (svc != MS_SVC_LIN_TSO && keyed && q.key >= p.sv_n_keys) { latch_error(st, E_VALUE_RANGE, q.key); continue; }
      if (svc != MS_SVC_LIN_TSO && !keyed) continue;
      uint32_t x[4] = {0, 0, 0, 0};
      if (svc == MS_SVC_SEQ_KV || svc == MS_SVC_LWW_KV)
        philox4x32_10(n_rep, e, (uint32_t)round, (uint32_t)(round >> 32), p.seed_lo, p.seed_hi, x);
      SvRep r;
      if (svc == MS_SVC_LIN_KV) {
        r.reply = false; r.otype = MS_T_ERROR; r.code = 0; r.value = 0;
        if (keyed) {
          if (q.key != ck) {
            if (cdirty) { p.sv_lin_has[ck] = chas ? 1 : 0; p.sv_lin_val[ck] = cval; }
            ck = q.key; chas = p.sv_lin_has[ck] != 0; cval = p.sv_lin_val[ck]; cdirty = false;
          }
          bool np_; uint32_t nv;
          kv_eval(chas, cval, q, false, r, np_, nv);
          if (r.reply) { cdirty = cdirty || np_ != chas || nv != cval; chas = np_; cval = nv; }
        }
      } else {
        service_handle(p, svc, q, x[3], r);
      }
      if (r.reply) {
        sm.vals[i] |= SV_REPLY | (r.code << 16) | r.otype;
        sm.keyB[pos] = r.value;
        n_rep++;
      }
    }
    if (cdirty) { p.sv_lin_has[ck] = chas ? 1 : 0; p.sv_lin_val[ck] = cval; }
  }
  __syncthreads();
}

#ifndef MS_ROUND_MINB2
#define MS_ROUND_MINB2 4
#endif
template <int CLS> struct ClsShape {
  static constexpr uint32_t cap = kClsLadder[CLS < 3 ? CLS : 2];
  static constexpr int nt = kClsThreads[CLS];
};

template <int CLS, int WL, bool FIX = false>
__global__ void __launch_bounds__(CLS == 3 ? 512 : 256, CLS == 3 ? 2 : MS_ROUND_MINB2) k_round(Params p, uint32_t cap_arg) {
  constexpr uint32_t cls = CLS;
  static_assert(!FIX || CLS < 3, "class 3 is sized by max_window");
  const uint32_t cap = FIX ? ClsShape<CLS>::cap : cap_arg;
  constexpr bool GS = (WL & 1) != 0;
  constexpr bool SV = (WL & 2) != 0;
  constexpr bool RF = (WL & 4) != 0;
  DevState* st = p.st;

#ifdef MS_EMUL
  unsigned char* smem_raw = simt::dyn_smem();
#else
  extern __shared__ __align__(16) unsigned char smem_raw[];
#endif
  uint64_t* reg1 = reinterpret_cast<uint64_t*>(smem_raw);
  uint32_t* keyB = reinterpret_cast<uint32_t*>(reg1 + cap + 1);
  uint32_t* vals = keyB + cap;
  uint16_t* tab = reinterpret_cast<uint16_t*>(vals + cap);
  uint16_t* meta = tab + 2 * (size_t)cap;
  uint16_t* ord = meta + cap;
  uint8_t* blk = reinterpret_cast<uint8_t*>(ord + cap);
  const RoundSmem sm{reg1, keyB, vals, tab, meta, ord, blk};
  uint64_t* keyA = reg1;
  uint64_t* aux = reg1;

  __shared__ uint64_t s_wtmp[34];
  __shared__ NetParams s_np;
  __shared__ uint32_t s_wcnt[17];
  __shared__ uint32_t s_misc[8];
  __shared__ uint32_t s_cnt[8];
  __shared__ uint64_t s_chunk;
  __shared__ uint16_t s_bstart[MAXB + 1];
  __shared__ uint16_t s_brank[MAXB];
  __shared__ uint16_t s_boff[MAXB + 1];
  __shared__ uint64_t s_bkeyA[MAXB];
  __shared__ uint64_t s_bbase[MAXB];
  __shared__ uint16_t s_S[MAXB + 1][MAXNB];
  __shared__ uint32_t s_nbbase[MAXNB];
  __shared__ uint32_t s_nbr[MAXNB];
  __shared__ uint4 s_gen[2];
  __shared__ uint64_t s_round0;
  __shared__ int64_t s_now0;
  __shared__ uint32_t s_go;

  const int tid = threadIdx.x, nt = FIX ? ClsShape<CLS>::nt : (int)blockDim.x, lane = tid & 31;
  if (tid == 0) {
    s_np = *p.np;
    const uint32_t so = ld_volatile_u32(&st->slot_open);
    __threadfence();
    const uint64_t r = *reinterpret_cast<const volatile uint64_t*>(&st->round);
    s_round0 = r;
    s_now0 = *reinterpret_cast<const volatile int64_t*>(&st->now);
    s_go = (so == slot_tag(r) && !round_skipped(p, st)) ? 1u : 0u;
  }
  __syncthreads();
  if (!s_go) return;
  const NetParams np = s_np;
  const int64_t now = s_now0;
  const uint64_t round = s_round0;
  const uint32_t T = p.n_inj_tickets + p.n_ep;
  const uint32_t row = (uint32_t)round & p.hist_mask;
  const uint32_t par = (uint32_t)round & 1u;
  const uint32_t my_big = st->cls_count[par][cls];
  const uint32_t my_count = my_big + st->cls_small[par][cls];
  const uint32_t* my_list = p.cls_list + ((size_t)par * 4 + cls) * p.t_max;
  const uint32_t tag = ((uint32_t)round & 0x7FFFu) + 1u;
  const bool need_rng = np.loss_thresh != 0 || np.dist != MS_DIST_CONSTANT;
  const uint64_t const_lat = (uint64_t)np.mean_ms * np.scale;
#ifdef MS_PHASE_TIMING
  const bool timing = p.phase_cycles != nullptr;
#else
  constexpr bool timing = false;
#endif
  long long t_prev = timing ? clock64() : 0;
#define PHASE_MARK(k)                                                                         \
  do {                                                                                        \
    if (timing && tid == 0) {                                                                 \
      const long long t_now = clock64();                                                      \
      atomicAdd((unsigned long long*)&p.phase_cycles[cls * 16 + (k)], (unsigned long long)(t_now - t_prev)); \
      t_prev = t_now;                                                                         \
    }                                                                                         \
  } while (0)
  if (tid == 0) s_misc[5] = atomicAdd(&st->cls_cursor[par][cls], 1u);

 for (;;) {
  __syncthreads();
  const uint32_t li = s_misc[5];
  if (tid < 5) s_misc[tid] = 0;
  if (tid < 8) s_cnt[tid] = 0;
  __syncthreads();
  if (li >= my_count) break;
  uint32_t next_li = 0;
  if (tid == 0) next_li = atomicAdd(&st->cls_cursor[par][cls], 1u);
  const uint32_t ticket = list_ticket(my_list, my_big, p.t_max, li);
  PHASE_MARK(0);
  if (timing && tid == 0) atomicAdd((unsigned long long*)&p.phase_cycles[cls * 16 + 15], 1ull);

  EmitCtx cx;
  cx.now = now;
  cx.round = round;
  cx.ticket = ticket;
  cx.idx_bias = 0;
  cx.chunk = 0;
  cx.n_recv = 0;
  cx.emitter = 0;
  cx.need_rng = need_rng;
  cx.const_lat = const_lat;
  cx.c_send_cl = cx.c_send_sv = cx.c_lost = cx.c_zero = 0;
  uint32_t c_recv_cl = 0, c_replies = 0;
  uint32_t n_ev_local = 0, n_em_local = 0;

  if (ticket < p.n_inj_tickets) {
    const uint32_t n_host = st->inj_count;
    const uint64_t tick = (uint64_t)(now / kTickNs);
    const uint32_t cur = st->sched_cursor;
    uint32_t hi = (tick + 1 < p.n_tick_off) ? p.tick_off[tick + 1] : p.n_sched;
    if (hi < cur) hi = cur;
    const uint32_t K = n_host + (hi - cur);
    const uint32_t chunk = (K + p.n_inj_tickets - 1) / p.n_inj_tickets;
    const uint32_t lo = min(ticket * chunk, K), hi_s = min(lo + chunk, K);
    const uint32_t n_local = hi_s - lo;
    n_ev_local = n_local; n_em_local = n_local;
    if (tid == 0) journal_claim(p, st, n_local, ticket, s_chunk);
    __syncthreads();
    cx.chunk = s_chunk;
    cx.emitter = kInjector;
    cx.idx_bias = lo;
    for (uint32_t base = 0; base < n_local; base += nt) {
      const uint32_t j = base + tid;
      const bool valid = j < n_local;
      Rec r;
      r.dest = 0; r.src = 0;
      if (valid) {
        const uint32_t g = lo + j;
        if (g < n_host) {
          const ms_msg m = p.inj_buf[g];
          r.src = m.src; r.dest = m.dest; r.msg_id = m.msg_id; r.in_reply_to = m.in_reply_to;
          r.tf = (uint32_t)m.type | ((uint32_t)m.flags << 16); r.p0 = m.p0; r.p1 = m.p1;
        } else {
          const ms_op op = p.sched[cur + (g - n_host)];
          r.src = op.src; r.dest = op.dest; r.msg_id = op.body.msg_id; r.in_reply_to = op.body.in_reply_to;
          r.tf = (uint32_t)op.body.type | ((uint32_t)op.body.flags << 16); r.p0 = op.body.p0; r.p1 = op.body.p1;
        }
      }
      emit_one(p, st, np, cx, valid, r, j, 0, false);
    }
  } else {
    const uint32_t e = ticket - p.n_inj_tickets;
    const uint8_t kind = p.kind[e];
    const uint32_t head = p.head[e];
    const bool has_c = p.cq && e < p.n_servers;
    const uint32_t chead = has_c ? p.head[p.cq + e] : 0u;
    uint32_t n_full = p.limit[e] - head;
    uint32_t n = n_full + (has_c ? p.limit[p.cq + e] - chead : 0u);
    if (kind & kRemoved) n = n_full = 0;
    if (n > cap || n > (e < p.n_servers ? p.max_window_s : p.max_window)) {
      if (tid == 0) latch_error(st, E_WINDOW_OVERFLOW, e);
      n = n_full = 0;
    }
    const uint4* myring = p.ring + ring_base(p, e) * 3;
    const uint32_t my_mask = ring_cap_of(p, e) - 1u;
    const Win win{myring, p.ring + p.cring_off + (size_t)e * p.ring_cap_s, head, chead, my_mask, n_full};
    const bool is_server = (kind == MS_KIND_SERVER);
    const bool bcast = !GS && is_server && p.workload == MS_W_BROADCAST;
    uint32_t n_timer = 0, fire_seq = 0, fire_p0 = 0;
    if constexpr (GS) {
      if (is_server && p.gs_init[e] && now >= p.gs_next_fire[e]) {
        n_timer = p.n_servers - 1;
        fire_seq = p.gs_fires[e] + 1;
      }
    }
    const uint32_t* mybits = (is_server && p.bitmap) ? p.bitmap + (size_t)e * p.bm_words : nullptr;
    const uint32_t deg = bcast ? nbr_count(p, e) : 0;
    const bool nb_smem = bcast && p.topology != MS_TOPO_TOTAL && deg <= MAXNB;
    if (nb_smem && tid < (int)deg) s_nbr[tid] = p.nbr[p.nbr_off[e] + tid];
    __syncthreads();

    {
      uint32_t err_val = 0xFFFFFFFFu;
      uint32_t snap_gone = 0xFFFFFFFFu;
      bool inj_srv = false;
      const bool nb4 = nb_smem && deg <= 4;
      const uint32_t nr0 = (nb4 && deg > 0) ? s_nbr[0] : 0xFFFFFFFFu, nr1 = (nb4 && deg > 1) ? s_nbr[1] : 0xFFFFFFFFu;
      const uint32_t nr2 = (nb4 && deg > 2) ? s_nbr[2] : 0xFFFFFFFFu, nr3 = (nb4 && deg > 3) ? s_nbr[3] : 0xFFFFFFFFu;
      for (int base = 0; base < (int)n; base += 2 * nt) {
        uint4 a[2], b[2], c[2];
#pragma unroll
        for (int q = 0; q < 2; q++) {
          const int i = base + q * nt + tid;
          if (i < (int)n) win_load(p, win, e, round, (uint32_t)i, a[q], b[q], c[q]);
        }
#pragma unroll
        for (int q = 0; q < 2; q++) {
          const int i = base + q * nt + tid;
          if (i >= (int)n) continue;
          const uint64_t rnd = (uint64_t)a[q].z | ((uint64_t)a[q].w << 32);
          keyA[i] = (rnd << 24) | (uint64_t)(a[q].y & 0xFFFFFFu);
          keyB[i] = a[q].x;
          const uint32_t src = b[q].x, tf = c[q].x, v = c[q].y;
          if (a[q].y < p.n_inj_tickets && src < p.n_servers) inj_srv = true;
          bool cut = false;
          if (np.pair_active && p.pair_bits)
            cut = (p.pair_bits[(size_t)e * p.pair_words + (src >> 5)] >> (src & 31)) & 1u;
          if (!cut && np.comp_active) {
            const uint32_t cs = p.comp[src], ce = p.comp[e];
            cut = cs != ce && cs != 0xFFFFFFFFu && ce != 0xFFFFFFFFu;
// ... 97 lines not shown
      const int c = ((int)n + nt - 1) / nt;
      const int nfull = (int)n_full;
      const int lo = min(tid * c, (int)n), hi = min(lo + c, (int)n);
      uint32_t nf = 0;
      uint32_t fmask = 0;
      const bool use_mask = c <= 32;
      if (lo < hi) {
        uint64_t pa = lo ? keyA[lo - 1] : 0ull;
        uint32_t pb = lo ? keyB[lo - 1] : 0u;
        for (int i = lo; i < hi; i++) {
          const uint64_t ka = keyA[i];
          const uint32_t kb = keyB[i];
          if (i == 0 || i == nfull || ka != pa || kb <= pb) { nf++; fmask |= 1u << ((i - lo) & 31); }
          pa = ka; pb = kb;
        }
      }
      uint32_t off = block_excl_scan_v(nf, &R, s_wcnt);
      if (R <= MAXB) {
        if (use_mask) {
          while (fmask) { s_bstart[off++] = (uint16_t)(lo + __ffs(fmask) - 1); fmask &= fmask - 1u; }
        } else {
          for (int i = lo; i < hi; i++)
            if (i == 0 || i == nfull || keyA[i] != keyA[i - 1] || keyB[i] <= keyB[i - 1]) s_bstart[off++] = (uint16_t)i;
        }
        if (tid == 0) s_bstart[R] = (uint16_t)n;
        __syncthreads();
        for (uint32_t b = tid; b < R; b += nt) {
          const uint32_t s0 = s_bstart[b];
          const uint64_t ka = keyA[s0];
          const uint32_t kb = keyB[s0];
          uint32_t rk = 0;
          for (uint32_t q = 0; q < R; q++) {
            const uint32_t sq = s_bstart[q];
            const uint64_t qa = keyA[sq];
            const uint32_t qb = keyB[sq];
            if (qa < ka || (qa == ka && (qb < kb || (qb == kb && q < b)))) rk++;
          }
          s_brank[b] = (uint16_t)rk;
          s_bkeyA[rk] = ka;
          s_boff[rk] = (uint16_t)(s_bstart[b + 1] - s0);
          s_bbase[rk] = ((uint64_t)kb << 32) | keyB[s_bstart[b + 1] - 1];
        }
        __syncthreads();
        if (tid == 0) {
          uint32_t acc = 0;
          bool ok = true;
          for (uint32_t q = 0; q < R; q++) {
            const uint32_t len = s_boff[q];
            s_boff[q] = (uint16_t)acc;
            acc += len;
            if (q) {
              const uint64_t pa = s_bkeyA[q - 1], ca = s_bkeyA[q];
              const uint32_t plast = (uint32_t)s_bbase[q - 1], cfirst = (uint32_t)(s_bbase[q] >> 32);
              if (!(pa < ca || (pa == ca && plast < cfirst))) ok = false;
            }
          }
          s_boff[R] = (uint16_t)acc;
          s_misc[1] = ok ? 1u : 0u;
          if (!ok && timing && atomicCAS((unsigned long long*)&p.phase_cycles[64], 0ull, 1ull) == 0ull) {
            unsigned long long* d = (unsigned long long*)p.phase_cycles + 65;
            d[0] = e; d[1] = n; d[2] = R; d[3] = round;
            for (uint32_t q = 0; q < R; q++) { d[4 + 2 * q] = s_bkeyA[q]; d[5 + 2 * q] = s_bbase[q]; }
          }
        }
        __syncthreads();
        use_blocks = s_misc[1] != 0;
      }
      if (use_blocks) {
        uint32_t bi = 0;
        if (lo < hi) {
          uint32_t l2 = 0, h2 = R;
          while (h2 - l2 > 1) { const uint32_t mid = (l2 + h2) >> 1; if (s_bstart[mid] <= (uint32_t)lo) l2 = mid; else h2 = mid; }
          bi = l2;
        }
        for (int i = lo; i < hi; i++) {
          while (bi + 1 < R && s_bstart[bi + 1] <= (uint32_t)i) bi++;
          const uint32_t rk = s_brank[bi];
          const uint32_t pos = s_boff[rk] + ((uint32_t)i - s_bstart[bi]);
          ord[pos] = (uint16_t)i;
          blk[pos] = (uint8_t)rk;
        }
        for (uint32_t b = tid; b < R; b += nt) {
          const uint64_t ka = s_bkeyA[b];
          s_bbase[b] = dense_base(p, st, ka >> 24, (uint32_t)(ka & 0xFFFFFFu));
        }
      } else {
        int np2 = 1;
        while (np2 < (int)n) np2 <<= 1;
        for (int i = tid; i < np2; i += nt) ord[i] = i < (int)n ? (uint16_t)i : (uint16_t)0xFFFF;
        __syncthreads();
        if (n > 1) block_bitonic_sort_idx(ord, keyA, keyB, np2);
        if (tid == 0 && n > 1) atomicAdd((unsigned long long*)&st->fallback_sorts, 1ull);
        if (timing && tid == 0 && n > 1) atomicAdd((unsigned long long*)&p.phase_cycles[cls * 16 + (R > MAXB ? 9 : 10)], 1ull);
      }
    }
    __syncthreads();
    PHASE_MARK(2);

    int npad = 1;
    while (npad < (int)n) npad <<= 1;
    const int tsz = 2 * npad;
    const uint32_t hshift = (uint32_t)__clz(tsz) + 1u;
#define TAB_SLOT(v) (((v) * 0x9E3779B1u) >> hshift)
    if (bcast && n > 0) {
      if (tsz >= 4) {
        uint64_t* t8 = reinterpret_cast<uint64_t*>(tab);
        for (int i = tid; i < (tsz >> 2); i += nt) t8[i] = 0xFFFFFFFFFFFFFFFFull;
      } else {
        for (int i = tid; i < tsz; i += nt) tab[i] = 0xFFFF;
      }
      __syncthreads();
      for (int pos = tid; pos < (int)n; pos += nt) {
        const uint32_t val = vals[ord[pos]];
        if (val & V_FRESH) {
          const uint32_t v = val & V_MASK;
          uint32_t h = TAB_SLOT(v);
          for (int probe = 0; probe < tsz; probe++) {
            uint32_t cur = *reinterpret_cast<volatile uint16_t*>(&tab[h]);
            if (cur == 0xFFFFu) {
              const uint32_t old = atomicCAS(&tab[h], (unsigned short)0xFFFF, (unsigned short)pos);
              if (old == 0xFFFFu) break;
              cur = old;
            }
            if ((vals[ord[cur]] & V_MASK) == v) {
              while ((uint32_t)pos < cur) {
                const uint32_t old = atomicCAS(&tab[h], (unsigned short)cur, (unsigned short)pos);
                if (old == cur) break;
                cur = old;
              }
              break;
            }
            h = (h + 1) & (tsz - 1);
          }
        }
      }
      __syncthreads();
    }
    if constexpr (RF) {
      if (is_server) {
        if (tid == 0) s_misc[2] = raft_step(p, st, e, now, round, win, n, sm);
        __syncthreads();
        n_timer = s_misc[2];
      }
    }
    if (kind == MS_KIND_GEN_CLIENT) {
      if (tid == 0) {
        Rec q;
        bool send;
        if constexpr (RF) send = kv_gen_step(p, st, e, now, round, myring, head, my_mask, n, ord, vals, q);
        else send = gen_step(p, st, e, now, round, myring, head, my_mask, n, ord, vals, q);
        if (send) {
          s_gen[0] = make_uint4(q.src, q.dest, q.msg_id, q.in_reply_to);
          if constexpr (RF) s_gen[1] = make_uint4(q.tf, q.p0, (uint32_t)q.p1, (uint32_t)(q.p1 >> 32));
          else s_gen[1] = make_uint4(q.tf, q.p0, 0u, 0u);
        }
        s_misc[2] = send ? 1u : 0u;
      }
      __syncthreads();
      n_timer = s_misc[2];
    }
    if constexpr (SV) {
      if (kind == MS_KIND_SERVICE) sv_step(p, st, e, round, win, n, sm);
    }
    for (int pos = tid; pos < (int)n; pos += nt) {
      const uint32_t i = ord[pos];
      uint32_t val = vals[i];
      bool is_new = false;
// ... 58 lines not shown
            snap[w] = x;
            cnt += __popc(x);
          }
          fire_p0 = block_sum_u32(cnt, s_wcnt);
        }
        for (uint32_t pos = tid; pos < n; pos += nt)
          if ((uint32_t)(aux[pos + 1] >> 48) != (uint32_t)(aux[pos] >> 48)) tab[(uint32_t)(aux[pos] >> 48)] = (uint16_t)pos;
        __syncthreads();
        uint32_t seg_lo = 0;
        for (uint32_t k = 0; k <= n_reads; k++) {
          const uint32_t seg_hi = k < n_reads ? (uint32_t)tab[k] : n;
          bool any_full = false;
          for (uint32_t pos = seg_lo + tid; pos < seg_hi; pos += nt) {
            const uint32_t i = ord[pos];
            const uint32_t val = vals[i], mt = meta[i];
            if (!(val & V_RECV) || (mt & M_REPLY)) continue;
            const uint32_t tc = (mt >> M_TC_SHIFT) & 7u;
            if (tc == GT_ADD || tc == GT_REPL_ONE) atomicOr(myset + ((val & V_MASK) >> 5), 1u << (val & 31));
            else if (tc == GT_REPL_FULL) any_full = true;
          }
          if (__syncthreads_or(any_full ? 1 : 0)) {
            for (uint32_t w = tid; w < p.bm_words; w += nt) {
              uint32_t acc = 0;
              for (uint32_t pos = seg_lo; pos < seg_hi; pos += 4) {
                uint32_t x[4] = {0u, 0u, 0u, 0u};
#pragma unroll
                for (uint32_t q = 0; q < 4; q++) {
                  if (pos + q >= seg_hi) continue;
                  const uint32_t i = ord[pos + q];
                  const uint32_t val = vals[i], mt = meta[i];
                  if ((val & V_RECV) && !(mt & M_REPLY) && ((mt >> M_TC_SHIFT) & 7u) == GT_REPL_FULL) {
                    const uint32_t srow = val & V_MASK;
                    const uint32_t* rows = p.gs_snap_sh[owner_of(srow / p.gs_slots, p.n_servers, p.n_shards)];
                    x[q] = __ldcg(rows + (size_t)srow * p.bm_words + w);
                  }
                }
                acc |= x[0] | x[1] | x[2] | x[3];
              }
              if (acc) myset[w] = __ldcg(myset + w) | acc;
            }
            __syncthreads();
          }
          if (k < n_reads) {
            uint32_t cnt = 0;
            for (uint32_t w = tid; w < p.bm_words; w += nt) cnt += __popc(__ldcg(myset + w));
            const uint32_t total = block_sum_u32(cnt, s_wcnt);
            if (tid == 0) keyB[seg_hi] = total;
            seg_lo = seg_hi + 1;
          }
        }
        __syncthreads();
      }
    }

    const bool mailed = (kind == MS_KIND_CLIENT || kind == MS_KIND_HOST);
    const bool agg_ok = nb_smem && n_new > 0 && !need_rng && const_lat == 0 && s_misc[3] == 0;
    const int agg_mode = !agg_ok ? 0 : (use_blocks ? 1 : (deg <= 4 ? 2 : 0));
    const bool agg = agg_mode != 0;
    const bool compact = agg && !np.any_removed && p.cq != 0;
    uint32_t* F01 = keyB;
    uint32_t* F23 = reinterpret_cast<uint32_t*>(tab);
    uint64_t f_total = 0;
    if (agg_mode == 2) {
      const int c = ((int)n + nt - 1) / nt;
      const int lo = min(tid * c, (int)n), hi = min(lo + c, (int)n);
      uint64_t acc = 0;
      for (int pos = lo; pos < hi; pos++) {
        const uint32_t i = ord[pos];
        const uint32_t ss = meta[i] & M_SRCSLOT;
        if ((vals[i] & V_FRESH) && ss >= 1 && ss <= 4) acc += 1ull << (16 * (ss - 1));
      }
      uint64_t run = block_excl_scan_v(acc, &f_total, s_wtmp);
      for (int pos = lo; pos < hi; pos++) {
        const uint32_t i = ord[pos];
        const uint32_t ss = meta[i] & M_SRCSLOT;
        F01[pos] = (uint32_t)run;
        F23[pos] = (uint32_t)(run >> 32);
        if ((vals[i] & V_FRESH) && ss >= 1 && ss <= 4) run += 1ull << (16 * (ss - 1));
      }
    }
    if (timing && tid == 0 && bcast && n_new > 0) atomicAdd((unsigned long long*)&p.phase_cycles[cls * 16 + (agg ? 11 : 12)], 1ull);
    if (timing && tid == 0 && n > 1) atomicAdd((unsigned long long*)&p.phase_cycles[cls * 16 + 13], (unsigned long long)R);
    if (tid == 32 % nt) {
      journal_claim(p, st, n_ev_local, ticket, s_chunk);
      s_cnt[3] = n_recv;
      s_cnt[6] = n - n_recv;
      if (mailed && n_recv) s_misc[0] = atomicAdd(&st->mail_count, n_recv);
    }
    if (agg && tid < (int)deg) {
      const uint32_t nb = s_nbr[tid];
      uint32_t acc = 0;
      if (agg_mode == 1) {
        for (uint32_t q = 0; q < R; q++) {
          s_S[q][tid] = (uint16_t)acc;
          const uint64_t ka = s_bkeyA[q];
          const uint32_t tk = (uint32_t)(ka & 0xFFFFFFu);
          if (tk >= p.n_inj_tickets && tk - p.n_inj_tickets == nb)
            acc += (uint32_t)(aux[s_boff[q + 1]] >> 48) - (uint32_t)(aux[s_boff[q]] >> 48);
        }
        s_S[R][tid] = (uint16_t)acc;
      } else {
        acc = (uint32_t)(f_total >> (16 * tid)) & 0xFFFFu;
      }
      const uint32_t total = n_new - acc;
      uint32_t base = 0;
      if (total) {
        const uint32_t o = owner_of(nb, p.n_servers, p.n_shards);
        const uint32_t ci = compact ? p.cq + nb : nb;
        base = atomicAdd(&p.tail_sh[o][ci], total);
        if (compact) {
          atomicAdd(&s_cnt[1], total);
          atomicAdd(&s_cnt[5], total);
        }
        if ((uint32_t)(base + total - p.head_sh[o][ci]) > ring_cap_of(p, nb)) latch_error(st, E_RING_OVERFLOW, nb);
      }
      s_nbbase[tid] = base;
    }
    __syncthreads();
    cx.chunk = s_chunk;
    cx.n_recv = n_recv;
    cx.emitter = e;
    const bool cl_ep = kind_is_client(kind);
    const uint32_t msg_id_base = (is_server && p.next_msg_id) ? p.next_msg_id[e] : 0;
    const uint32_t set_before = (is_server && p.set_count) ? p.set_count[e] : 0;
    NbrList L;
    L.nl = nb_smem ? s_nbr : nullptr;
    L.deg = deg;
    PHASE_MARK(5);

    const bool full_recv = p.jlevel >= 2 || mailed || !use_blocks;
    for (uint32_t pos = tid; pos < n; pos += nt) {
      const uint32_t i = ord[pos];
      const uint32_t val = vals[i];
      if (!(val & V_RECV)) continue;
      const uint32_t k = (uint32_t)(aux[pos] >> 32) & 0xFFFFu;
      const uint32_t mt = meta[i];
      const uint32_t sslot = mt & M_SRCSLOT;
      if (full_recv || !nb_smem || sslot == 0) {
        Rec m = win_rec(p, win, e, round, i);
        const uint64_t id = (use_blocks ? s_bbase[blk[pos]] : dense_base(p, st, m.round, m.ticket)) + m.idx;
        journal_raw(p, cx.chunk + k, id, true, m);
        const bool cl = cl_ep || (m.src >= p.n_servers && kind_is_client(p.kind[m.src]));
        if (cl) c_recv_cl++;
        if (kind == MS_KIND_SIM_CLIENT && ((m.tf >> 16) & MS_F_REPLY)) c_replies++;
        if (mailed) {
          const uint32_t mpos = s_misc[0] + k;
          if (mpos >= p.mail_cap) {
            latch_error(st, E_MAIL_OVERFLOW, e);
          } else {
            uint4* dst = reinterpret_cast<uint4*>(p.mail) + (size_t)mpos * 3;
            st_v4(dst + 0, make_uint4((uint32_t)id, (uint32_t)(id >> 32), (uint32_t)now, (uint32_t)((uint64_t)now >> 32)));
            st_v4(dst + 1, make_uint4(m.src, m.dest, m.msg_id, m.in_reply_to));
            st_v4(dst + 2, make_uint4(m.tf, m.p0, (uint32_t)m.p1, (uint32_t)(m.p1 >> 32)));
          }
        }
      } else {
        const uint64_t id = s_bbase[blk[pos]] + keyB[i];
        const uint64_t vrec = id | RECV_BIT;
        if (p.jlevel)
          st_v4(p.jraw + ((cx.chunk + k) & p.jmask),
                make_uint4((uint32_t)vrec, (uint32_t)(vrec >> 32), s_nbr[sslot - 1], e));
      }
    }
    const bool own_map = agg_mode != 2 && n_emit_msgs <= 2u * cap;
    if (own_map) {
      for (uint32_t pos = tid; pos < n; pos += nt) {
        const uint32_t e0 = (uint32_t)aux[pos], e1 = (uint32_t)aux[pos + 1];
        for (uint32_t q = e0; q < e1; q++) tab[q] = (uint16_t)pos;
      }
      __syncthreads();
    }
    for (uint32_t base = 0; base < n_emit; base += nt) {
      const uint32_t j = base + tid;
      const bool valid = j < n_emit;
      Rec r;
      r.dest = 0; r.src = e;
      uint32_t direct = 0;
      bool has_direct = false;
      bool fast = false;
      bool timer_emission = false;
      if constexpr (GS) {
        if (valid && j < n_timer) {
          timer_emission = true;
          r.dest = j < e ? j : j + 1;
          r.msg_id = 0; r.in_reply_to = 0; r.tf = MS_T_REPLICATE_FULL; r.p0 = fire_p0; r.p1 = fire_seq;
        }
      }
      if constexpr (RF) {
        if (is_server && valid && j < n_timer) {
          timer_emission = true;
          const uint4* at = p.rf_stage + ((size_t)e * p.rf_stage_cap + j) * 3;
          const uint4 a = at[0], b = at[1];
          r.src = a.x; r.dest = a.y; r.msg_id = a.z; r.in_reply_to = a.w;
          r.tf = b.x; r.p0 = b.y; r.p1 = (uint64_t)b.z | ((uint64_t)b.w << 32);
        }
      }
      if (kind == MS_KIND_GEN_CLIENT && valid && j < n_timer) {
        timer_emission = true;
        const uint4 a = s_gen[0], b = s_gen[1];
        r.src = a.x; r.dest = a.y; r.msg_id = a.z; r.in_reply_to = a.w;
        r.tf = b.x; r.p0 = b.y; r.p1 = 0;
        if constexpr (RF) r.p1 = (uint64_t)b.z | ((uint64_t)b.w << 32);
      }
      if (valid && !timer_emission) {
        const uint32_t jm = j - n_timer;
        uint32_t pos;
        if (own_map) {
          pos = tab[jm];
        } else {
          uint32_t lo = 0, hi = n;
          while (hi - lo > 1) { const uint32_t mid = (lo + hi) >> 1; if ((uint32_t)aux[mid] <= jm) lo = mid; else hi = mid; }
          pos = lo;
        }
        const uint64_t a0 = aux[pos];
        const uint32_t k = jm - (uint32_t)a0;
        const uint32_t my_emit = (uint32_t)aux[pos + 1] - (uint32_t)a0;
        const uint32_t new_before = (uint32_t)(a0 >> 48);
        const uint32_t i = ord[pos];
        const uint32_t val = vals[i];
        const uint32_t mt = meta[i];
        const bool gossip = bcast && ((mt >> M_TC_SHIFT) & 7u) == TC_BROADCAST && !(mt & M_REPLY) &&
                            !((mt & M_HAS_ID) && k == my_emit - 1);
        if (gossip && nb_smem) {
          const uint32_t ss = mt & M_SRCSLOT;
          const uint32_t js = (ss && k >= ss - 1) ? k + 1 : k;
          r.dest = s_nbr[js];
          r.msg_id = 0; r.in_reply_to = 0; r.tf = MS_T_BROADCAST; r.p0 = val & V_MASK; r.p1 = 0;
          if (agg_mode == 1) {
            direct = s_nbbase[js] + new_before - s_S[blk[pos]][js];
            has_direct = true;
          } else if (agg_mode == 2) {
            const uint32_t f = js < 2 ? (F01[pos] >> (16 * js)) : (F23[pos] >> (16 * (js - 2)));
            direct = s_nbbase[js] + new_before - (f & 0xFFFFu);
            has_direct = true;
          }
          fast = compact;
        } else {
          uint4 va, vb, vc;
          win_load(p, win, e, round, i, va, vb, vc);
          MsgView w;
          w.src = vb.x; w.msg_id = vb.z; w.tf = vc.x; w.p0 = vc.y;
          const uint64_t p1 = (uint64_t)vc.z | ((uint64_t)vc.w << 32);
          bool svc_emission = false;
          if constexpr (SV) {
            if (kind == MS_KIND_SERVICE) {
              svc_emission = true;
              r.src = e; r.dest = w.src; r.msg_id = 0; r.in_reply_to = w.msg_id;
              r.tf = (val & 0xFFFFu) | ((uint32_t)MS_F_REPLY << 16);
              r.p0 = (val >> 16) & 0xFFu;
              r.p1 = keyB[pos];
            }
          }
          if (svc_emission) {
          } else if constexpr (GS) {
            const uint32_t tc = (mt >> M_TC_SHIFT) & 7u;
            r.src = e; r.dest = w.src; r.msg_id = 0; r.in_reply_to = w.msg_id; r.p0 = 0; r.p1 = 0;
            uint32_t otype = MS_T_ERROR;
            if (tc == GT_INIT) otype = MS_T_INIT_OK;
            else if (tc == GT_ADD) otype = MS_T_ADD_OK;
            else if (tc == GT_READ) { otype = MS_T_READ_OK; r.p0 = keyB[pos]; }
            else r.p0 = 10;
            r.tf = otype | ((uint32_t)MS_F_REPLY << 16);
          } else {
          (void)node_emit(p, e, w, k, my_emit, jm, msg_id_base, set_before, new_before, p1, r, L);
          }
        }
      }
      if (fast) {
        r.round = round; r.ticket = ticket; r.idx = j;
        journal_raw(p, cx.chunk + n_recv + j, j, false, r);
        uint4* ring_o = p.ring_sh[owner_of(r.dest, p.n_servers, p.n_shards)];
        st_v4(cring_slot(p, ring_o, r.dest, direct), make_uint4(j, ticket, (uint32_t)round, r.p0));
      }
      if (__any_sync(FULL, valid && !fast)) emit_one(p, st, np, cx, valid && !fast, r, j, direct, has_direct);
    }
    if (tid == 0 && is_server) {
      if (p.workload == MS_W_ECHO && p.next_msg_id && n_emit) p.next_msg_id[e] = msg_id_base + n_emit;
      if constexpr (!GS) {
      if (p.set_count && n_new) p.set_count[e] = set_before + n_new;
      } else {
        int64_t nf = p.gs_next_fire[e];
        if (n_timer) {
          nf += (int64_t)p.gs_interval_ms * kTickNs;
          p.gs_fires[e] = fire_seq;
          p.gs_tag[e * p.gs_slots + (fire_seq & (p.gs_slots - 1))] = fire_seq;
        }
        if (s_misc[2]) { p.gs_init[e] = 1; nf = now; }
        p.gs_next_fire[e] = nf;
      }
      if (n > st->max_window_seen) atomicMax(&st->max_window_seen, n);
    }
  }

  PHASE_MARK(6);
  {
    uint32_t cnt[6] = {cx.c_send_cl, cx.c_send_sv, c_recv_cl, cx.c_lost, cx.c_zero, c_replies};
    constexpr int at[6] = {0, 1, 2, 4, 5, 7};
    if (__any_sync(FULL, (cnt[0] | cnt[1] | cnt[2] | cnt[3] | cnt[4] | cnt[5]) != 0)) {
#pragma unroll
      for (int q = 0; q < 6; q++) {
#pragma unroll
        for (int d = 16; d > 0; d >>= 1) cnt[q] += __shfl_xor_sync(FULL, cnt[q], d);
        if (lane == 0 && cnt[q]) atomicAdd(&s_cnt[at[q]], cnt[q]);
      }
      if (lane == 0 && cnt[2]) atomicAdd(&s_cnt[3], 0u - cnt[2]);
    }
  }
  __syncthreads();
  if (tid < 8 && s_cnt[tid]) {
    const uint32_t v = s_cnt[tid];
    if (tid == 0) atomicAdd((unsigned long long*)&st->stats[2], (unsigned long long)v);
    else if (tid == 1) atomicAdd((unsigned long long*)&st->stats[4], (unsigned long long)v);
    else if (tid == 2) atomicAdd((unsigned long long*)&st->stats[3], (unsigned long long)v);
    else if (tid == 3) atomicAdd((unsigned long long*)&st->stats[5], (unsigned long long)v);
    else if (tid == 4) atomicAdd((unsigned long long*)&st->lost, (unsigned long long)v);
    else if (tid == 6) atomicAdd((unsigned long long*)&st->part_drops, (unsigned long long)v);
    else if (tid == 7) atomicAdd((unsigned long long*)&st->client_replies, (unsigned long long)v);
  }
  if (tid == 0) {
    if (n_ev_local >= (1u << 23) || n_em_local >= (1u << 24)) latch_error(st, E_ID_RANGE, ticket);
    p.rt_chunk[(size_t)row * p.t_max + ticket] = cx.chunk;
    const uint64_t entry = ((uint64_t)tag << 48) | (s_cnt[5] ? (1ull << 47) : 0ull) |
                           ((uint64_t)(n_ev_local & 0x7FFFFFu) << 24) | (uint64_t)(n_em_local & 0xFFFFFFu);
    __stcg(reinterpret_cast<unsigned long long*>(p.rt_cnt + (size_t)row * p.t_max + ticket),
           (unsigned long long)entry);
    s_misc[4] = (!p.split_commit && atomicAdd(&st->done, 1u) == T - 1) ? 1u : 0u;
    s_misc[5] = next_li;
  }
  __syncthreads();
  PHASE_MARK(7);
  if (s_misc[4]) {
    commit_round(p, st, s_wtmp);
    PHASE_MARK(8);
  }
 }
#undef PHASE_MARK
#undef TAB_SLOT
}

struct JChunk {
  const RoundMeta* m;
  uint64_t g0, cnt, chunk, send_base;
};
__device__ __forceinline__ bool journal_chunk(const Params& p, uint64_t r0, uint64_t c, uint64_t first, uint64_t count,
                                              JChunk& j) {
  const uint64_t r = r0 + c / p.t_max;
  const uint32_t t = (uint32_t)(c % p.t_max);
  const uint32_t row = (uint32_t)r & p.hist_mask;
  const RoundMeta* m = p.rmeta + row;
  if (m->round != r || t >= m->n_tickets) return false;
  if (owner_of_ticket(t, p.n_inj_tickets, p.n_servers, p.n_shards) != p.shard_id) return false;
  const uint32_t* ev = p.rt_ev + (size_t)row * p.t_max;
  const uint64_t off = ev[t];
  const uint64_t end = (t + 1 < m->n_tickets) ? ev[t + 1] : m->ev_total;
  if (end == off) return false;
  const uint64_t g0 = m->ev_base + off;
  const uint64_t cnt = end - off;
  if (g0 + cnt <= first || g0 >= first + count) return false;
  j = JChunk{m, g0, cnt, p.rt_chunk[(size_t)row * p.t_max + t], m->id_base + p.rt_em[(size_t)row * p.t_max + t]};
  return true;
}

__device__ __forceinline__ void event_rec(uint64_t g, bool recv, int64_t tnow, uint64_t id, uint4 raw, uint4& a, uint4& b) {
  const uint64_t eid = g | (recv ? MS_EVENT_RECV : 0ull);
  a = make_uint4((uint32_t)eid, (uint32_t)(eid >> 32), (uint32_t)tnow, (uint32_t)((uint64_t)tnow >> 32));
  b = make_uint4((uint32_t)id, (uint32_t)(id >> 32), raw.z, raw.w);
}

__device__ __forceinline__ uint64_t jfmt8_word(uint64_t id, uint64_t id_ref, bool recv, uint4 raw, bool& bad) {
  const uint64_t d = id - id_ref;
  if (id < id_ref || d >= (1ull << 31) || raw.z > 0xFFFFu || raw.w > 0xFFFFu) bad = true;
  return (recv ? RECV_BIT : 0ull) | ((uint64_t)(raw.z & 0xFFFFu) << 47) | ((uint64_t)(raw.w & 0xFFFFu) << 31) |
         (d & 0x7FFFFFFFull);
}

__global__ void k_journal_expand(Params p, uint64_t r0, uint32_t n_rounds, uint64_t first, uint64_t count,
                                 uint4* out_ev, uint4* out_body) {
  const uint32_t lane = threadIdx.x & 31;
  const uint64_t warp_global = ((uint64_t)blockIdx.x * blockDim.x + threadIdx.x) >> 5;
  const uint64_t n_warps = ((uint64_t)gridDim.x * blockDim.x) >> 5;
  const uint64_t n_chunks = (uint64_t)n_rounds * p.t_max;
  for (uint64_t c = warp_global; c < n_chunks; c += n_warps) {
    JChunk j;
    if (!journal_chunk(p, r0, c, first, count, j)) continue;
    const uint64_t g0 = j.g0, cnt = j.cnt, chunk = j.chunk, send_base = j.send_base;
    const int64_t tnow = j.m->now;
    for (uint64_t k = lane; k < cnt; k += 32) {
      const uint64_t g = g0 + k;
      if (g < first || g >= first + count) continue;
      const uint4 raw = p.jraw[(chunk + k) & p.jmask];
      const uint64_t v = (uint64_t)raw.x | ((uint64_t)raw.y << 32);
      const bool recv = (v & RECV_BIT) != 0;
      const uint64_t id = recv ? (v & ~RECV_BIT) : send_base + v;
      uint4 e0, e1;
      event_rec(g, recv, tnow, id, raw, e0, e1);
      uint4* o = out_ev + (g - first) * 2;
      st_v4(o + 0, e0);
      st_v4(o + 1, e1);
      if (out_body) {
        const uint4* b = p.jbody + ((chunk + k) & p.jmask) * 2;
        const uint4 b0 = b[0], b1 = b[1];
        uint4* ob = out_body + (g - first) * 2;
        st_v4(ob + 0, make_uint4((uint32_t)id, (uint32_t)(id >> 32), b0.z, b0.w));
        st_v4(ob + 1, b1);
      }
    }
  }
}

struct StreamMark {
  uint64_t round, next_event, raw_base;
  uint32_t error, pad;
};
struct StreamPlan {
  uint64_t first, count, r0, n_rounds;
  uint64_t journal_drained, drain_round, jraw_drained;
  uint32_t overflow, more;
  unsigned long long local_n;
  uint64_t hist[2][3];
  uint64_t pad;
  StreamMark mark[2];
};
static_assert(sizeof(StreamPlan) == 128 + 2 * 32, "StreamPlan is initialised from the host");

__global__ void k_stream_mark(Params p, StreamPlan* plan, uint32_t parity) {
  if (threadIdx.x || blockIdx.x) return;
  const DevState* st = p.st;
  StreamMark mk;
  mk.round = st->round;
  mk.next_event = st->next_event;
  mk.raw_base = p.rmeta[(uint32_t)mk.round & p.hist_mask].raw_base;
  mk.error = st->error;
  mk.pad = 0;
  plan->mark[parity] = mk;
}

__global__ void k_stream_plan(Params p, StreamPlan* plan, uint64_t cap_events, uint32_t cap_rounds, ms_jround* rows,
                              uint32_t format, uint32_t parity) {
  if (threadIdx.x || blockIdx.x) return;
  const StreamMark mk = plan->mark[parity];
  const uint64_t first = plan->journal_drained;
  uint64_t count = mk.next_event > first ? mk.next_event - first : 0;
  if (count > cap_events) count = cap_events;
  const uint64_t r0 = plan->drain_round;
  uint64_t r1 = r0, covered = first;
  while (r1 < mk.round) {
    const RoundMeta* m = p.rmeta + ((uint32_t)r1 & p.hist_mask);
    if (m->round != r1 || m->ev_base >= first + count) break;
    if (r1 - r0 >= cap_rounds) break;
    ms_jround row;
    row.round = r1; row.time_ns = m->now; row.ev_base = m->ev_base;
    row.id_ref = (format == MS_JFMT_4 && p.n_shards <= 1) ? m->id_base
                                                          : (m->id_base > (1ull << 30) ? m->id_base - (1ull << 30) : 0ull);
    rows[r1 - r0] = row;
    covered = m->ev_base + m->ev_total;
    r1++;
  }
  if (count > (covered > first ? covered - first : 0)) count = covered > first ? covered - first : 0;
  plan->first = first; plan->count = count; plan->r0 = r0; plan->n_rounds = r1 - r0;
  plan->overflow = 0;
  plan->local_n = 0;
}

template <int FMT>
__global__ void k_journal_pack(Params p, StreamPlan* plan, unsigned char* out) {
  const uint64_t first = plan->first, count = plan->count, r0 = plan->r0;
  const uint32_t n_rounds = (uint32_t)plan->n_rounds;
  if (count == 0) return;
  const uint32_t lane = threadIdx.x & 31;
  const uint64_t warp_global = ((uint64_t)blockIdx.x * blockDim.x + threadIdx.x) >> 5;
  const uint64_t n_warps = ((uint64_t)gridDim.x * blockDim.x) >> 5;
  const uint64_t n_chunks = (uint64_t)n_rounds * p.t_max;
  bool bad = false;
  for (uint64_t c = warp_global; c < n_chunks; c += n_warps) {
    JChunk j;
    if (!journal_chunk(p, r0, c, first, count, j)) continue;
    const RoundMeta* m = j.m;
    const uint64_t g0 = j.g0, cnt = j.cnt, chunk = j.chunk, send_base = j.send_base;
    const uint64_t id_ref = m->id_base > (1ull << 30) ? m->id_base - (1ull << 30) : 0ull;
    const int64_t tnow = m->now;
    uint64_t slot0 = 0;
    const uint64_t k_lo = g0 < first ? first - g0 : 0, k_hi = g0 + cnt > first + count ? first + count - g0 : cnt;
    if (p.n_shards > 1) {
      if (lane == 0) slot0 = atomicAdd(&plan->local_n, (unsigned long long)(k_hi - k_lo));
      slot0 = __shfl_sync(FULL, slot0, 0);
    }
    for (uint64_t k = lane; k < cnt; k += 32) {
      const uint64_t g = g0 + k;
      if (g < first || g >= first + count) continue;
      const uint4 raw = p.jraw[(chunk + k) & p.jmask];
      const uint64_t v = (uint64_t)raw.x | ((uint64_t)raw.y << 32);
      const bool recv = (v & RECV_BIT) != 0;
      const uint64_t id = recv ? (v & ~RECV_BIT) : send_base + v;
      if (p.n_shards > 1) {
        const uint64_t at = slot0 + (k - k_lo);
        if (FMT == 32) {
          uint4* o = reinterpret_cast<uint4*>(out) + at * 2;
          event_rec(g, recv, tnow, id, raw, o[0], o[1]);
        } else {
          const uint64_t eid = g | (recv ? MS_EVENT_RECV : 0ull);
          const uint64_t w = jfmt8_word(id, id_ref, recv, raw, bad);
          reinterpret_cast<uint4*>(out)[at] = make_uint4((uint32_t)eid, (uint32_t)(eid >> 32), (uint32_t)w, (uint32_t)(w >> 32));
        }
        continue;
      }
      if (FMT == 8) {
        reinterpret_cast<unsigned long long*>(out)[g - first] = jfmt8_word(id, id_ref, recv, raw, bad);
      } else if (FMT == 4) {
        uint32_t w;
        if (recv) {
          const uint64_t d = m->id_base - 1ull - id;
          if (id >= m->id_base || d >= (1ull << 31)) bad = true;
          w = 0x80000000u | (uint32_t)(d & 0x7FFFFFFFull);
        } else {
          if (raw.z > 0x7FFFu || raw.w > 0xFFFFu) bad = true;
          w = ((raw.z & 0x7FFFu) << 16) | (raw.w & 0xFFFFu);
        }
        reinterpret_cast<uint32_t*>(out)[g - first] = w;
      } else if (FMT == 12) {
        if (id >= (1ull << 47) || raw.z > 0xFFFFFFu || raw.w > 0xFFFFFFu) bad = true;
        uint32_t* o = reinterpret_cast<uint32_t*>(out) + (g - first) * 3;
        o[0] = (uint32_t)id;
        o[1] = (uint32_t)((id >> 32) & 0x7FFFu) | (recv ? 0x8000u : 0u) | ((raw.z & 0xFFFFu) << 16);
        o[2] = ((raw.z >> 16) & 0xFFu) | (raw.w << 8);
      } else {
        uint4* o = reinterpret_cast<uint4*>(out) + (g - first) * 2;
        event_rec(g, recv, tnow, id, raw, o[0], o[1]);
      }
    }
  }
  if (bad) atomicOr(&plan->overflow, 1u);
}

__global__ void k_stream_finish(Params p, StreamPlan* plan, ms_jbatch* hdr, uint32_t format, uint32_t parity) {
  if (threadIdx.x || blockIdx.x) return;
  const StreamMark mk = plan->mark[parity];
  const DevState* st = p.st;
  plan->journal_drained = plan->first + plan->count;
  uint64_t dr = plan->drain_round;
  while (dr < mk.round) {
    const RoundMeta* m = p.rmeta + ((uint32_t)dr & p.hist_mask);
    if (m->round != dr || m->ev_base + m->ev_total > plan->journal_drained) break;
    dr++;
  }
  plan->drain_round = dr;
  plan->jraw_drained = dr < mk.round ? p.rmeta[(uint32_t)dr & p.hist_mask].raw_base : mk.raw_base;
  plan->more = mk.next_event > plan->journal_drained ? 1u : 0u;
  plan->hist[parity][0] = plan->journal_drained;
  plan->hist[parity][1] = plan->drain_round;
  plan->hist[parity][2] = plan->jraw_drained;
  ms_jbatch b;
  b.first_event = plan->first; b.n_events = p.n_shards > 1 ? (uint64_t)plan->local_n : plan->count; b.n_rounds = plan->n_rounds;
  b.now = st->now; b.round = st->round; b.next_event = mk.next_event;
  b.format = (p.n_shards > 1 && format != MS_JFMT_EVENT) ? (uint32_t)MS_JFMT_16 : format;
  b.overflow = plan->overflow; b.more = plan->more; b.error = st->error | mk.error;
  b.range_events = plan->count;
  *hdr = b;
  __threadfence_system();
}

__global__ void k_stream_apply(Params p, const StreamPlan* plan, uint32_t parity) {
  if (threadIdx.x || blockIdx.x) return;
  DevState* st = p.st;
  const uint64_t a = plan->hist[parity][0], b = plan->hist[parity][1], c = plan->hist[parity][2];
  if (a > st->journal_drained) st->journal_drained = a;
  if (b > st->drain_round) st->drain_round = b;
  if (c > st->jraw_drained) st->jraw_drained = c;
}

}

extern "C" {

typedef void (*msk_round_fn)(msd::Params, uint32_t);
static msk_round_fn msk_round_kernel(uint32_t family, int cls, bool fixed = false) {
  if (fixed && (family & 7u) == 0 && cls < 3) {
    static const msk_round_fn fx[3] = {msd::k_round<0, 0, true>, msd::k_round<1, 0, true>, msd::k_round<2, 0, true>};
    return fx[cls];
  }
  static const msk_round_fn tab[8][4] = {
      {msd::k_round<0, 0>, msd::k_round<1, 0>, msd::k_round<2, 0>, msd::k_round<3, 0>},
      {msd::k_round<0, 1>, msd::k_round<1, 1>, msd::k_round<2, 1>, msd::k_round<3, 1>},
      {msd::k_round<0, 2>, msd::k_round<1, 2>, msd::k_round<2, 2>, msd::k_round<3, 2>},
      {msd::k_round<0, 3>, msd::k_round<1, 3>, msd::k_round<2, 3>, msd::k_round<3, 3>},
      {msd::k_round<0, 4>, msd::k_round<1, 4>, msd::k_round<2, 4>, msd::k_round<3, 4>},
      {nullptr, nullptr, nullptr, nullptr},
      {msd::k_round<0, 6>, msd::k_round<1, 6>, msd::k_round<2, 6>, msd::k_round<3, 6>},
      {nullptr, nullptr, nullptr, nullptr}};
  return tab[family & 7u][cls];
}

cudaError_t msk_round_smem_attr(size_t bytes) {
  cudaError_t e = cudaSuccess;
  for (uint32_t f = 0; f < 8 && e == cudaSuccess; f++)
    for (int c = 0; c < 4 && e == cudaSuccess; c++)
      if (msk_round_kernel(f, c))
        e = cudaFuncSetAttribute(msk_round_kernel(f, c), cudaFuncAttributeMaxDynamicSharedMemorySize, (int)bytes);
  for (int c = 0; c < 3 && e == cudaSuccess; c++)
    e = cudaFuncSetAttribute(msk_round_kernel(0, c, true), cudaFuncAttributeMaxDynamicSharedMemorySize, (int)bytes);
  return e;
}

size_t msk_round_smem_bytes(uint32_t cap) { return (size_t)cap * 25 + 32; }

void msk_set_bit(uint32_t* words, size_t word, uint32_t bit, cudaStream_t s) {
  MS_LAUNCH(msd::k_set_bit, 1, 1, 0, s, words, word, bit);
}

int msk_round_occupancy(int threads, size_t smem) {
  int nb = 0;
// ... 94 lines not shown
```

maelstrom_b200/engine.py:

```python
import ctypes as C

import numpy as np

from . import _lib
from ._lib import Body, Config, EVENT_DTYPE, JBODY_DTYPE, MSG_DTYPE, OP_DTYPE

WORKLOADS = {"echo": 0, "broadcast": 1, "g-set": 2, "lin-kv": 3, "txn-list-append": 4, "txn-list-append-tree": 5}
TOPOLOGIES = {"grid": 0, "line": 1, "total": 2, "tree": 3, "tree2": 3, "tree3": 4, "tree4": 5}
DISTS = {"constant": 0, "uniform": 1, "exponential": 2}
KIND_SERVER, KIND_CLIENT, KIND_HOST, KIND_SIM_CLIENT, KIND_SERVICE = 0, 1, 2, 3, 4
SERVICES = ("lin-kv", "seq-kv", "lww-kv", "lin-tso")
TYPES = dict(init=1, init_ok=2, error=3, echo=10, echo_ok=11, topology=20, topology_ok=21,
             broadcast=22, broadcast_ok=23, read=24, read_ok=25, add=30, add_ok=31,
             replicate_one=32, replicate_full=33, write=40, write_ok=41, cas=42, cas_ok=43, ts=44, ts_ok=45,
             request_vote=50, request_vote_res=51, append_entries=52, append_entries_res=53,
             txn=60, txn_ok=61)
TYPE_NAMES = {v: k for k, v in TYPES.items()}
F_MSG_ID, F_REPLY, F_CREATE, F_APPENDS = 1, 2, 4, 8
RECV_BIT = 1 << 63


class SimError(RuntimeError):
    def __init__(self, code, text):
        RuntimeError.__init__(self, "maelstrom_b200 error %d: %s" % (code, text))
# ... 200 lines not shown
        return self._chk(self.L.ms_journal_open(self.h, path.encode()))

    def journal_close(self):
        return self._chk(self.L.ms_journal_close(self.h))

    def drain(self, cap=1 << 20, bodies=True):
        parts = self._stash + [self._drain_now(cap, bodies)]
        self._stash = []
        ev = np.concatenate([p[0] for p in parts])
        bd = np.concatenate([p[1] for p in parts]) if bodies else None
        if getattr(self, "_jdecoder", None) is not None and len(ev):
            self._jdecoder.note(ev)
        return ev, bd

    def _drain_now(self, cap=1 << 20, bodies=True):
        evs, bds = [], []
        while True:
            ev = np.zeros(cap, dtype=EVENT_DTYPE)
            bd = np.zeros(cap, dtype=JBODY_DTYPE) if bodies else None
            n = C.c_size_t(0)
            self._chk(self.L.ms_journal_drain(self.h, ev.ctypes.data,
                                              bd.ctypes.data if bodies else None, cap, C.byref(n)))
            if n.value == 0:
                break
            evs.append(ev[:n.value])
            if bodies:
                bds.append(bd[:n.value])
        ev = np.concatenate(evs) if evs else np.zeros(0, dtype=EVENT_DTYPE)
        bd = (np.concatenate(bds) if bds else np.zeros(0, dtype=JBODY_DTYPE)) if bodies else None
        return ev, bd

    def run_streamed(self, until_ns, sink=None, fmt=_lib.JFMT_8, buf_events=0, decode=False, decoder=None):
        tot = [0, 0]
        err = []
        if decode and fmt == _lib.JFMT_4 and decoder is None:
            if getattr(self, "_jdecoder", None) is None:
                self._jdecoder = JournalDecoder()
            decoder = self._jdecoder

        def _cb(ctx, bp, rounds_p, events_p):
            try:
                b = bp.contents
                n = int(b.n_events)
                tot[0] += n
                tot[1] += n * int(b.format)
                if sink is not None:
                    rounds = np.ctypeslib.as_array(C.cast(rounds_p, C.POINTER(C.c_uint8)),
                                                   (int(b.n_rounds) * 32,)).view(_lib.JROUND_DTYPE)
                    if decode and decoder is not None:
                        ev = decoder.decode_raw(bp, rounds_p, events_p, n)
                    elif decode:
                        ev = np.zeros(n, dtype=EVENT_DTYPE)
                        self._chk(self.L.ms_journal_decode(bp, rounds_p, events_p, ev.ctypes.data))
                    else:
                        raw = np.ctypeslib.as_array(C.cast(events_p, C.POINTER(C.c_uint8)), (n * int(b.format),))
                        ev = (raw.view("<u4") if b.format == 4 else
                              raw.view("<u8") if b.format == 8 else raw.view("<u4").reshape(n, 3) if b.format == 12
                              else raw.view("<u8").reshape(n, 2) if b.format == 16 else raw.view(EVENT_DTYPE))
                    info = {k: int(getattr(b, k)) for k, _ in _lib.JBatch._fields_}
                    sink(info, rounds, ev)
                return 0
            except Exception as e:
                err.append(e)
                return 1

        cb = _lib.JOURNAL_SINK(_cb)
        rc = self.L.ms_run_streamed(self.h, until_ns, fmt, buf_events, cb, None)
        if err:
            raise err[0]
        self._chk(rc)
        return tot[0], tot[1]

    def journal_written(self):
        return int(self.L.ms_journal_written(self.h))

    def stats(self):
        out = np.zeros(9, dtype=np.uint64)
        self._chk(self.L.ms_stats(self.h, out.ctypes.data))
        keys = ("send-count", "recv-count", "msg-count")
        return {cls: {k: int(out[i * 3 + j]) for j, k in enumerate(keys)}
                for i, cls in enumerate(("all", "clients", "servers"))}

    def counters(self):
        out = np.zeros(8, dtype=np.uint64)
        self._chk(self.L.ms_counters(self.h, out.ctypes.data))
        names = ("rounds", "sends", "recvs", "launches", "lost", "partition_drops", "max_window", "fallback_sorts")
        return {k: int(v) for k, v in zip(names, out)}

    RING_FIELDS = ("tail", "limit", "head", "ctail", "climit", "chead")

    def ring_counters(self):
        S = self.n_nodes
        out = np.zeros(6 * S, dtype=np.uint64)
        self._chk(self.L.ms_ring_counters(self.h, out.ctypes.data, out.size))
        return {k: out[i * S:(i + 1) * S].astype(np.uint32) for i, k in enumerate(self.RING_FIELDS)}

    def set_origin(self, round=0, msg_id=0, event_id=0, ring_pos=0, ring_stride=0):
        return self._chk(self.L.ms_set_origin(self.h, round, msg_id, event_id, ring_pos & 0xFFFFFFFF,
                                              ring_stride & 0xFFFFFFFF))

    def timer_begin(self):
        return self._chk(self.L.ms_timer_begin(self.h))

    def timer_end(self):
        ms = C.c_double(0)
        self._chk(self.L.ms_timer_end(self.h, C.byref(ms)))
        return ms.value

    def profile(self, enable=True):
        return self._chk(self.L.ms_profile(self.h, 1 if enable else 0))

    def profile_read(self):
        ms = C.c_double(0)
        n = C.c_uint64(0)
        self._chk(self.L.ms_profile_read(self.h, C.byref(ms), C.byref(n)))
        return ms.value, int(n.value)

    def phase_cycles(self, enable=True):
        out = np.zeros(64, dtype=np.uint64)
        self._chk(self.L.ms_debug_phase_cycles(self.h, 1 if enable else 0, out.ctypes.data))
        return out.reshape(4, 16)

    def drain_into(self, ev_ptr, cap, body_ptr=None):
        n = C.c_size_t(0)
        self._chk(self.L.ms_journal_drain(self.h, ev_ptr, body_ptr, cap, C.byref(n)))
        return int(n.value)

    def node_set(self, node):
        n = self.L.ms_node_set(self.h, node, None, 0)
        out = np.zeros(max(n, 1), dtype=np.uint32)
        self.L.ms_node_set(self.h, node, out.ctypes.data, n)
        return out[:n]

    def client_replies(self):
        return int(self.L.ms_client_replies(self.h))

    def undeliverable(self):
        return int(self.L.ms_undeliverable(self.h))

    RAFT_FIELDS = ("state", "term", "voted_for", "commit_index", "last_applied", "leader", "log_size", "kv_size")

    def raft_state(self, node):
        out = np.zeros(8, dtype=np.uint64)
        self._chk(self.L.ms_raft_state(self.h, node, out.ctypes.data))
        d = dict(zip(self.RAFT_FIELDS, (int(x) for x in out)))
        d["voted_for"] -= 1
        d["leader"] -= 1
        return d


HIST_TYPES = ("invoke", "ok", "fail", "info")
HF_KV_READ, HF_KV_WRITE, HF_KV_CAS = 2, 3, 4
H_NEMESIS = 0xFFFFFFFF
HF_NEM_ONE, HF_NEM_MAJORITY, HF_NEM_MINORITY_THIRD, HF_NEM_STOP = 5, 6, 7, 8
HF_NEM_MAJORITIES_RING = 9
NEM_ONE, NEM_MAJORITY, NEM_MINORITY_THIRD = 1, 2, 4
NEM_MAJORITIES_RING = 16


def nemesis_grudge(seed, cluster, g, op, target):
    out = np.zeros(max(g, 1), dtype=np.uint32)
    rc = _lib.lib().ms_nemesis_grudge(seed & 0xFFFFFFFF, seed >> 32, cluster, g, op, target, out.ctypes.data)
    if rc < 0:
        raise SimError(rc, _lib.lib().ms_last_error(None).decode())
    return out[:g]


def kv_history(records, first_client, group_clients):
    out = {}
# ... 23 lines not shown
```

Measured before the change: 11.86 billion.

## Compress journal raw records to 8-byte narrow entries with wide fallback

Journal raw records drop from 16 to 8 bytes in the common case. Receive records store a 31-bit delta from the round id_base plus the source, and send records store src/dest with the id implied by position. Chunks whose deltas could overflow (mailed, non-block path, resolved tickets, or large deltas) fall back to a 'wide' two-unit encoding flagged in the chunk's high bit, and a wide_chunks counter is exposed. The goal is to halve journal write bandwidth in the simulation kernel, at the cost of more complex encode/decode logic and a host staging buffer sized in units.

After: 12.05 billion (median of 6 runs). 1.6% higher.

```diff
diff --git a/include/maelstrom_b200.h b/include/maelstrom_b200.h
--- a/include/maelstrom_b200.h
+++ b/include/maelstrom_b200.h
@@ -247,6 +247,7 @@
 int      ms_raft_state(ms_sim* sim, uint32_t node, uint64_t out[8]);
 
 int ms_counters(ms_sim* sim, uint64_t out[8]);
+int ms_counters_n(ms_sim* sim, uint64_t* out, uint32_t n);
 
 int ms_ring_counters(ms_sim* sim, uint64_t* out, uint32_t n);
 
diff --git a/integration/java/maelstrom/b200/Native.java b/integration/java/maelstrom/b200/Native.java
--- a/integration/java/maelstrom/b200/Native.java
+++ b/integration/java/maelstrom/b200/Native.java
@@ -56,6 +56,7 @@
   public static native long undeliverable(long h);
   public static native int raftState(long h, int node, ByteBuffer out8);
   public static native int counters(long h, ByteBuffer out8);
+  public static native int countersN(long h, ByteBuffer out, int n);
   public static native int ringCounters(long h, ByteBuffer out, int n);
   public static native int setOrigin(long h, long round, long msgId, long eventId, int ringPos, int ringStride);
   public static native int shardHandles(long h, ByteBuffer blob512);
diff --git a/maelstrom_b200/_lib.py b/maelstrom_b200/_lib.py
--- a/maelstrom_b200/_lib.py
+++ b/maelstrom_b200/_lib.py
@@ -121,6 +121,7 @@
     "ms_undeliverable": (C.c_uint64, [_P]),
     "ms_raft_state": (C.c_int, [_P, C.c_uint32, _P]),
     "ms_counters": (C.c_int, [_P, _P]),
+    "ms_counters_n": (C.c_int, [_P, _P, C.c_uint32]),
     "ms_ring_counters": (C.c_int, [_P, _P, C.c_uint32]),
     "ms_set_origin": (C.c_int, [_P, C.c_uint64, C.c_uint64, C.c_uint64, C.c_uint32, C.c_uint32]),
     "ms_timer_begin": (C.c_int, [_P]),
diff --git a/maelstrom_b200/csrc/ms_device.cuh b/maelstrom_b200/csrc/ms_device.cuh
--- a/maelstrom_b200/csrc/ms_device.cuh
+++ b/maelstrom_b200/csrc/ms_device.cuh
@@ -68,6 +68,7 @@
   uint32_t cls_cursor[2][4];
   uint64_t idle_wake;
   int64_t  nem_next;
+  uint64_t wide_chunks;
 };
 
 struct RoundMeta {
diff --git a/maelstrom_b200/csrc/ms_engine.cu b/maelstrom_b200/csrc/ms_engine.cu
--- a/maelstrom_b200/csrc/ms_engine.cu
+++ b/maelstrom_b200/csrc/ms_engine.cu
@@ -413,7 +413,7 @@
     const size_t n = (size_t)std::min<uint64_t>(avail, cap);
     if (n == 0) return MS_OK;
     if (!stage_ev) {
-      stage_cap = (size_t)std::min<uint64_t>(P.jmask + 1, 1ull << 22);
+      stage_cap = (size_t)std::min<uint64_t>((P.jmask + 1) / 2, 1ull << 22);
       CK(cudaMalloc(&stage_ev, stage_cap * 32));
       if (cfg.journal_level >= 2) CK(cudaMalloc(&stage_body, stage_cap * 32));
     }
@@ -682,7 +682,7 @@
     CK(cudaMalloc(&ptr, J * 16));
     s->allocs.push_back(ptr);
     P.jraw = (uint4*)ptr;
-    P.jmask = J - 1;
+    P.jmask = 2 * J - 1;
     if (c.journal_level >= 2) {
       CK(cudaMalloc(&ptr, J * 32));
       s->allocs.push_back(ptr);
@@ -1942,8 +1942,11 @@
   return MS_OK;
 }
 
-int ms_counters(ms_sim* s, uint64_t out[8]) {
-  std::lock_guard<std::mutex> g(s->mu);
+int ms_counters(ms_sim* s, uint64_t out[8]) { return ms_counters_n(s, out, 8); }
+
+int ms_counters_n(ms_sim* s, uint64_t* out, uint32_t n) {
+  std::lock_guard<std::mutex> g(s->mu);
+  if (!out || n < 8) { set_err("ms_counters_n: out needs at least 8 entries"); return MS_ERR_ARG; }
   out[0] = s->hs.rounds_run;
   out[1] = s->hs.stats[2] + s->hs.stats[4];
   out[2] = s->hs.stats[3] + s->hs.stats[5];
@@ -1952,6 +1955,7 @@
   out[5] = s->hs.part_drops;
   out[6] = s->hs.max_window_seen;
   out[7] = s->hs.fallback_sorts;
+  if (n > 8) out[8] = s->hs.wide_chunks;
   return MS_OK;
 }
 
diff --git a/maelstrom_b200/csrc/ms_jni.c b/maelstrom_b200/csrc/ms_jni.c
--- a/maelstrom_b200/csrc/ms_jni.c
+++ b/maelstrom_b200/csrc/ms_jni.c
@@ -173,6 +173,7 @@
 jlong FN(undeliverable)(JNIEnv* env, jclass c, jlong h) { (void)env; (void)c; return (jlong)ms_undeliverable(H(h)); }
 jint FN(raftState)(JNIEnv* env, jclass c, jlong h, jint node, jobject out8) { (void)c; return ms_raft_state(H(h), (uint32_t)node, (uint64_t*)BUF(out8)); }
 jint FN(counters)(JNIEnv* env, jclass c, jlong h, jobject out8) { (void)c; return ms_counters(H(h), (uint64_t*)BUF(out8)); }
+jint FN(countersN)(JNIEnv* env, jclass c, jlong h, jobject out, jint n) { (void)c; return ms_counters_n(H(h), (uint64_t*)BUF(out), (uint32_t)n); }
 jint FN(ringCounters)(JNIEnv* env, jclass c, jlong h, jobject out, jint n) { (void)c; return ms_ring_counters(H(h), (uint64_t*)BUF(out), (uint32_t)n); }
 jint FN(setOrigin)(JNIEnv* env, jclass c, jlong h, jlong round, jlong msg_id, jlong event_id, jint ring_pos, jint ring_stride) {
   (void)env; (void)c;
diff --git a/maelstrom_b200/csrc/ms_kernels.cu b/maelstrom_b200/csrc/ms_kernels.cu
--- a/maelstrom_b200/csrc/ms_kernels.cu
+++ b/maelstrom_b200/csrc/ms_kernels.cu
@@ -217,22 +217,89 @@
   uint32_t c_send_cl, c_send_sv, c_lost, c_zero;
 };
 
-__device__ __forceinline__ void journal_raw(const Params& p, uint64_t pos, uint64_t id_or_idx, bool recv,
-                                            const Rec& r) {
+constexpr uint64_t kWideChunk = 1ull << 63;
+
+__device__ __forceinline__ void st_u64(unsigned long long* p, uint64_t v) {
+#ifdef MS_EMUL
+  *p = v;
+#else
+  asm volatile("st.global.L1::no_allocate.u64 [%0], %1;" ::"l"(p), "l"(v) : "memory");
+#endif
+}
+
+__device__ __forceinline__ uint4* jbody_at(const Params& p, uint64_t chunk, uint64_t k) {
+  return p.jbody + ((((chunk & ~kWideChunk) >> 1) + k) & (p.jmask >> 1)) * 2;
+}
+
+__device__ __forceinline__ void jraw_put(const Params& p, uint64_t chunk, uint64_t k, bool recv, uint64_t id_or_idx,
+                                         uint64_t id_base, uint32_t src, uint32_t dest) {
+  unsigned long long* u = reinterpret_cast<unsigned long long*>(p.jraw);
+  if (chunk & kWideChunk) {
+    const uint64_t v = id_or_idx | (recv ? RECV_BIT : 0ull);
+    st_v4(reinterpret_cast<uint4*>(u + (((chunk & ~kWideChunk) + 2 * k) & p.jmask)),
+          make_uint4((uint32_t)v, (uint32_t)(v >> 32), src, dest));
+  } else {
+    const uint32_t w0 = recv ? 0x80000000u | (uint32_t)(id_base - 1ull - id_or_idx) : src;
+    st_u64(u + ((chunk + k) & p.jmask), (uint64_t)w0 | ((uint64_t)(recv ? src : dest) << 32));
+  }
+}
+
+__device__ __forceinline__ void jraw_put_recv_narrow(const Params& p, uint64_t chunk, uint64_t k, uint32_t delta,
+                                                     uint32_t src) {
+  st_u64(reinterpret_cast<unsigned long long*>(p.jraw) + ((chunk + k) & p.jmask),
+         (uint64_t)(0x80000000u | delta) | ((uint64_t)src << 32));
+}
+
+struct JRec {
+  uint64_t id;
+  uint32_t src, dest;
+  bool recv;
+};
+__device__ __forceinline__ JRec jraw_get(const Params& p, uint64_t chunk, uint64_t k, uint64_t n_recv, uint32_t owner,
+                                         uint64_t send_base, uint64_t id_base) {
+  const unsigned long long* u = reinterpret_cast<const unsigned long long*>(p.jraw);
+  JRec e;
+  if (chunk & kWideChunk) {
+    const uint4 raw = *reinterpret_cast<const uint4*>(u + (((chunk & ~kWideChunk) + 2 * k) & p.jmask));
+    const uint64_t v = (uint64_t)raw.x | ((uint64_t)raw.y << 32);
+    e.recv = (v & RECV_BIT) != 0;
+    e.id = e.recv ? (v & ~RECV_BIT) : send_base + v;
+    e.src = raw.z;
+    e.dest = raw.w;
+  } else {
+    const uint64_t w = u[(chunk + k) & p.jmask];
+    e.recv = k < n_recv;
+    e.id = e.recv ? id_base - 1ull - (w & 0x7FFFFFFFull) : send_base + (k - n_recv);
+    e.src = e.recv ? (uint32_t)(w >> 32) : (uint32_t)w;
+    e.dest = e.recv ? owner : (uint32_t)(w >> 32);
+  }
+  return e;
+}
+
+__device__ __forceinline__ void journal_raw(const Params& p, const EmitCtx& cx, uint64_t k, bool recv,
+                                            uint64_t id_or_idx, uint64_t id_base, const Rec& r) {
   if (p.jlevel == 0) return;
-  const uint64_t v = id_or_idx | (recv ? RECV_BIT : 0ull);
-  st_v4(p.jraw + (pos & p.jmask), make_uint4((uint32_t)v, (uint32_t)(v >> 32), r.src, r.dest));
+  jraw_put(p, cx.chunk, k, recv, id_or_idx, id_base, r.src, r.dest);
   if (p.jlevel >= 2) {
-    uint4* b = p.jbody + (pos & p.jmask) * 2;
+    const uint64_t v = id_or_idx | (recv ? RECV_BIT : 0ull);
+    uint4* b = jbody_at(p, cx.chunk, k);
     st_v4(b + 0, make_uint4((uint32_t)v, (uint32_t)(v >> 32), r.msg_id, r.in_reply_to));
     st_v4(b + 1, make_uint4(r.tf, r.p0, (uint32_t)r.p1, (uint32_t)(r.p1 >> 32)));
   }
 }
 
-__device__ __forceinline__ void journal_claim(const Params& p, DevState* st, uint32_t n, uint32_t ticket, uint64_t& chunk) {
-  chunk = (n && p.jlevel) ? atomicAdd((unsigned long long*)&st->jraw_cursor, (unsigned long long)n) : 0ull;
-  if (n && p.jlevel && !p.jdiscard && chunk + n - st->jraw_drained > p.jmask + 1)
-    latch_error(st, E_JOURNAL_OVERFLOW, ticket);
+__device__ __forceinline__ void journal_claim(const Params& p, DevState* st, uint32_t n, bool wide, uint32_t ticket,
+                                              uint64_t& chunk, uint32_t& n_wide) {
+  chunk = 0;
+  if (!n || !p.jlevel) return;
+  wide = wide || p.jlevel >= 2;
+  const uint64_t units = wide ? 2ull * n : (n + 1ull) & ~1ull;
+  chunk = atomicAdd((unsigned long long*)&st->jraw_cursor, (unsigned long long)units);
+  if (!p.jdiscard && chunk + units - st->jraw_drained > p.jmask + 1) latch_error(st, E_JOURNAL_OVERFLOW, ticket);
+  if (wide) {
+    chunk |= kWideChunk;
+    n_wide++;
+  }
 }
 
 __device__ __forceinline__ uint32_t ld_volatile_u32(const uint32_t* p) {
@@ -305,7 +372,7 @@
     const bool cl = (r.src >= p.n_servers && r.src < p.n_ep && kind_is_client(p.kind[r.src])) ||
                     (r.dest >= p.n_servers && r.dest < p.n_ep && kind_is_client(p.kind[r.dest]));
     const uint64_t lat = cl ? 0ull : (cx.need_rng ? latency_ms(np, x) : cx.const_lat);
-    journal_raw(p, cx.chunk + cx.n_recv + local_idx, local_idx, false, r);
+    journal_raw(p, cx, cx.n_recv + local_idx, false, local_idx, 0, r);
     if (cl) cx.c_send_cl++; else cx.c_send_sv++;
     if (undeliverable) {
       atomicAdd((unsigned long long*)&st->undeliverable, 1ull);
@@ -1508,11 +1575,14 @@
   __shared__ uint32_t s_misc[8];
   __shared__ uint32_t s_cnt[8];
   __shared__ uint64_t s_chunk;
+  __shared__ uint64_t s_idb;
+  __shared__ uint32_t s_nwide;
   __shared__ uint16_t s_bstart[MAXB + 1];
   __shared__ uint16_t s_brank[MAXB];
   __shared__ uint16_t s_boff[MAXB + 1];
   __shared__ uint64_t s_bkeyA[MAXB];
   __shared__ uint64_t s_bbase[MAXB];
+  __shared__ uint32_t s_bdelta[MAXB];
   __shared__ uint16_t s_S[MAXB + 1][MAXNB];
   __shared__ uint32_t s_nbbase[MAXNB];
   __shared__ uint32_t s_nbr[MAXNB];
@@ -1560,11 +1630,15 @@
     }                                                                                         \
   } while (0)
   if (tid == 0) s_misc[5] = atomicAdd(&st->cls_cursor[par][cls], 1u);
+  if (tid == 0) {
+    s_idb = p.rmeta[row].id_base;
+    s_nwide = 0;
+  }
 
  for (;;) {
   __syncthreads();
   const uint32_t li = s_misc[5];
-  if (tid < 5) s_misc[tid] = 0;
+  if (tid < 8 && tid != 5) s_misc[tid] = 0;
   if (tid < 8) s_cnt[tid] = 0;
   __syncthreads();
   if (li >= my_count) break;
@@ -1599,7 +1673,7 @@
     const uint32_t lo = min(ticket * chunk, K), hi_s = min(lo + chunk, K);
     const uint32_t n_local = hi_s - lo;
     n_ev_local = n_local; n_em_local = n_local;
-    if (tid == 0) journal_claim(p, st, n_local, ticket, s_chunk);
+    if (tid == 0) journal_claim(p, st, n_local, false, ticket, s_chunk, s_nwide);
     __syncthreads();
     cx.chunk = s_chunk;
     cx.emitter = kInjector;
@@ -1863,7 +1937,10 @@
         }
         for (uint32_t b = tid; b < R; b += nt) {
           const uint64_t ka = s_bkeyA[b];
-          s_bbase[b] = dense_base(p, st, ka >> 24, (uint32_t)(ka & 0xFFFFFFu));
+          const uint64_t base = dense_base(p, st, ka >> 24, (uint32_t)(ka & 0xFFFFFFu));
+          s_bbase[b] = base;
+          s_bdelta[b] = (uint32_t)(s_idb - 1ull - base);
+          if ((ka & 0xFFFFFFu) == kResolvedTicket) s_misc[6] = 1;
         }
       } else {
         int np2 = 1;
@@ -2088,7 +2165,8 @@
     if (timing && tid == 0 && bcast && n_new > 0) atomicAdd((unsigned long long*)&p.phase_cycles[cls * 16 + (agg ? 11 : 12)], 1ull);
     if (timing && tid == 0 && n > 1) atomicAdd((unsigned long long*)&p.phase_cycles[cls * 16 + 13], (unsigned long long)R);
     if (tid == 32 % nt) {
-      journal_claim(p, st, n_ev_local, ticket, s_chunk);
+      const bool wide = n_recv && (mailed || !use_blocks || s_misc[6] || s_idb - 1ull - s_bbase[0] >= (1ull << 31));
+      journal_claim(p, st, n_ev_local, wide, ticket, s_chunk, s_nwide);
       s_cnt[3] = n_recv;
       s_cnt[6] = n - n_recv;
       if (mailed && n_recv) s_misc[0] = atomicAdd(&st->mail_count, n_recv);
@@ -2145,7 +2223,7 @@
       if (full_recv || !nb_smem || sslot == 0) {
         Rec m = win_rec(p, win, e, round, i);
         const uint64_t id = (use_blocks ? s_bbase[blk[pos]] : dense_base(p, st, m.round, m.ticket)) + m.idx;
-        journal_raw(p, cx.chunk + k, id, true, m);
+        journal_raw(p, cx, k, true, id, s_idb, m);
         const bool cl = cl_ep || (m.src >= p.n_servers && kind_is_client(p.kind[m.src]));
         if (cl) c_recv_cl++;
         if (kind == MS_KIND_SIM_CLIENT && ((m.tf >> 16) & MS_F_REPLY)) c_replies++;
@@ -2161,11 +2239,11 @@
           }
         }
       } else {
-        const uint64_t id = s_bbase[blk[pos]] + keyB[i];
-        const uint64_t vrec = id | RECV_BIT;
-        if (p.jlevel)
-          st_v4(p.jraw + ((cx.chunk + k) & p.jmask),
-                make_uint4((uint32_t)vrec, (uint32_t)(vrec >> 32), s_nbr[sslot - 1], e));
+        const uint32_t b = blk[pos];
+        if (p.jlevel) {
+          if (cx.chunk & kWideChunk) jraw_put(p, cx.chunk, k, true, s_bbase[b] + keyB[i], 0, s_nbr[sslot - 1], e);
+          else jraw_put_recv_narrow(p, cx.chunk, k, s_bdelta[b] - keyB[i], s_nbr[sslot - 1]);
+        }
       }
     }
     const bool own_map = agg_mode != 2 && n_emit_msgs <= 2u * cap;
@@ -2274,7 +2352,7 @@
       }
       if (fast) {
         r.round = round; r.ticket = ticket; r.idx = j;
-        journal_raw(p, cx.chunk + n_recv + j, j, false, r);
+        journal_raw(p, cx, n_recv + j, false, j, 0, r);
         uint4* ring_o = p.ring_sh[owner_of(r.dest, p.n_servers, p.n_shards)];
         st_v4(cring_slot(p, ring_o, r.dest, direct), make_uint4(j, ticket, (uint32_t)round, r.p0));
       }
@@ -2340,13 +2418,18 @@
     PHASE_MARK(8);
   }
  }
+  if (tid == 0 && s_nwide) atomicAdd((unsigned long long*)&st->wide_chunks, (unsigned long long)s_nwide);
 #undef PHASE_MARK
 #undef TAB_SLOT
 }
 
 struct JChunk {
   const RoundMeta* m;
-  uint64_t g0, cnt, chunk, send_base;
+  uint64_t g0, cnt, chunk, send_base, n_recv;
+  uint32_t owner;
+  __device__ __forceinline__ JRec get(const Params& p, uint64_t k) const {
+    return jraw_get(p, chunk, k, n_recv, owner, send_base, m->id_base);
+  }
 };
 __device__ __forceinline__ bool journal_chunk(const Params& p, uint64_t r0, uint64_t c, uint64_t first, uint64_t count,
                                               JChunk& j) {
@@ -2357,26 +2440,29 @@
   if (m->round != r || t >= m->n_tickets) return false;
   if (owner_of_ticket(t, p.n_inj_tickets, p.n_servers, p.n_shards) != p.shard_id) return false;
   const uint32_t* ev = p.rt_ev + (size_t)row * p.t_max;
+  const uint32_t* em = p.rt_em + (size_t)row * p.t_max;
   const uint64_t off = ev[t];
   const uint64_t end = (t + 1 < m->n_tickets) ? ev[t + 1] : m->ev_total;
   if (end == off) return false;
   const uint64_t g0 = m->ev_base + off;
   const uint64_t cnt = end - off;
   if (g0 + cnt <= first || g0 >= first + count) return false;
-  j = JChunk{m, g0, cnt, p.rt_chunk[(size_t)row * p.t_max + t], m->id_base + p.rt_em[(size_t)row * p.t_max + t]};
+  const uint64_t n_em = ((t + 1 < m->n_tickets) ? em[t + 1] : m->em_total) - em[t];
+  j = JChunk{m, g0, cnt, p.rt_chunk[(size_t)row * p.t_max + t], m->id_base + em[t], cnt - n_em,
+             t < p.n_inj_tickets ? kInjector : t - p.n_inj_tickets};
   return true;
 }
 
-__device__ __forceinline__ void event_rec(uint64_t g, bool recv, int64_t tnow, uint64_t id, uint4 raw, uint4& a, uint4& b) {
-  const uint64_t eid = g | (recv ? MS_EVENT_RECV : 0ull);
+__device__ __forceinline__ void event_rec(uint64_t g, int64_t tnow, const JRec& e, uint4& a, uint4& b) {
+  const uint64_t eid = g | (e.recv ? MS_EVENT_RECV : 0ull);
   a = make_uint4((uint32_t)eid, (uint32_t)(eid >> 32), (uint32_t)tnow, (uint32_t)((uint64_t)tnow >> 32));
-  b = make_uint4((uint32_t)id, (uint32_t)(id >> 32), raw.z, raw.w);
-}
-
-__device__ __forceinline__ uint64_t jfmt8_word(uint64_t id, uint64_t id_ref, bool recv, uint4 raw, bool& bad) {
-  const uint64_t d = id - id_ref;
-  if (id < id_ref || d >= (1ull << 31) || raw.z > 0xFFFFu || raw.w > 0xFFFFu) bad = true;
-  return (recv ? RECV_BIT : 0ull) | ((uint64_t)(raw.z & 0xFFFFu) << 47) | ((uint64_t)(raw.w & 0xFFFFu) << 31) |
+  b = make_uint4((uint32_t)e.id, (uint32_t)(e.id >> 32), e.src, e.dest);
+}
+
+__device__ __forceinline__ uint64_t jfmt8_word(const JRec& e, uint64_t id_ref, bool& bad) {
+  const uint64_t d = e.id - id_ref;
+  if (e.id < id_ref || d >= (1ull << 31) || e.src > 0xFFFFu || e.dest > 0xFFFFu) bad = true;
+  return (e.recv ? RECV_BIT : 0ull) | ((uint64_t)(e.src & 0xFFFFu) << 47) | ((uint64_t)(e.dest & 0xFFFFu) << 31) |
          (d & 0x7FFFFFFFull);
 }
 
@@ -2389,25 +2475,22 @@
   for (uint64_t c = warp_global; c < n_chunks; c += n_warps) {
     JChunk j;
     if (!journal_chunk(p, r0, c, first, count, j)) continue;
-    const uint64_t g0 = j.g0, cnt = j.cnt, chunk = j.chunk, send_base = j.send_base;
+    const uint64_t g0 = j.g0, cnt = j.cnt;
     const int64_t tnow = j.m->now;
     for (uint64_t k = lane; k < cnt; k += 32) {
       const uint64_t g = g0 + k;
       if (g < first || g >= first + count) continue;
-      const uint4 raw = p.jraw[(chunk + k) & p.jmask];
-      const uint64_t v = (uint64_t)raw.x | ((uint64_t)raw.y << 32);
-      const bool recv = (v & RECV_BIT) != 0;
-      const uint64_t id = recv ? (v & ~RECV_BIT) : send_base + v;
+      const JRec e = j.get(p, k);
       uint4 e0, e1;
-      event_rec(g, recv, tnow, id, raw, e0, e1);
+      event_rec(g, tnow, e, e0, e1);
       uint4* o = out_ev + (g - first) * 2;
       st_v4(o + 0, e0);
       st_v4(o + 1, e1);
       if (out_body) {
-        const uint4* b = p.jbody + ((chunk + k) & p.jmask) * 2;
+        const uint4* b = jbody_at(p, j.chunk, k);
         const uint4 b0 = b[0], b1 = b[1];
         uint4* ob = out_body + (g - first) * 2;
-        st_v4(ob + 0, make_uint4((uint32_t)id, (uint32_t)(id >> 32), b0.z, b0.w));
+        st_v4(ob + 0, make_uint4((uint32_t)e.id, (uint32_t)(e.id >> 32), b0.z, b0.w));
         st_v4(ob + 1, b1);
       }
     }
@@ -2482,7 +2565,7 @@
     JChunk j;
     if (!journal_chunk(p, r0, c, first, count, j)) continue;
     const RoundMeta* m = j.m;
-    const uint64_t g0 = j.g0, cnt = j.cnt, chunk = j.chunk, send_base = j.send_base;
+    const uint64_t g0 = j.g0, cnt = j.cnt;
     const uint64_t id_ref = m->id_base > (1ull << 30) ? m->id_base - (1ull << 30) : 0ull;
     const int64_t tnow = m->now;
     uint64_t slot0 = 0;
@@ -2494,24 +2577,23 @@
     for (uint64_t k = lane; k < cnt; k += 32) {
       const uint64_t g = g0 + k;
       if (g < first || g >= first + count) continue;
-      const uint4 raw = p.jraw[(chunk + k) & p.jmask];
-      const uint64_t v = (uint64_t)raw.x | ((uint64_t)raw.y << 32);
-      const bool recv = (v & RECV_BIT) != 0;
-      const uint64_t id = recv ? (v & ~RECV_BIT) : send_base + v;
+      const JRec e = j.get(p, k);
+      const bool recv = e.recv;
+      const uint64_t id = e.id;
       if (p.n_shards > 1) {
         const uint64_t at = slot0 + (k - k_lo);
         if (FMT == 32) {
           uint4* o = reinterpret_cast<uint4*>(out) + at * 2;
-          event_rec(g, recv, tnow, id, raw, o[0], o[1]);
+          event_rec(g, tnow, e, o[0], o[1]);
         } else {
           const uint64_t eid = g | (recv ? MS_EVENT_RECV : 0ull);
-          const uint64_t w = jfmt8_word(id, id_ref, recv, raw, bad);
+          const uint64_t w = jfmt8_word(e, id_ref, bad);
           reinterpret_cast<uint4*>(out)[at] = make_uint4((uint32_t)eid, (uint32_t)(eid >> 32), (uint32_t)w, (uint32_t)(w >> 32));
         }
         continue;
       }
       if (FMT == 8) {
-        reinterpret_cast<unsigned long long*>(out)[g - first] = jfmt8_word(id, id_ref, recv, raw, bad);
+        reinterpret_cast<unsigned long long*>(out)[g - first] = jfmt8_word(e, id_ref, bad);
       } else if (FMT == 4) {
         uint32_t w;
         if (recv) {
@@ -2519,19 +2601,19 @@
           if (id >= m->id_base || d >= (1ull << 31)) bad = true;
           w = 0x80000000u | (uint32_t)(d & 0x7FFFFFFFull);
         } else {
-          if (raw.z > 0x7FFFu || raw.w > 0xFFFFu) bad = true;
-          w = ((raw.z & 0x7FFFu) << 16) | (raw.w & 0xFFFFu);
+          if (e.src > 0x7FFFu || e.dest > 0xFFFFu) bad = true;
+          w = ((e.src & 0x7FFFu) << 16) | (e.dest & 0xFFFFu);
         }
         reinterpret_cast<uint32_t*>(out)[g - first] = w;
       } else if (FMT == 12) {
-        if (id >= (1ull << 47) || raw.z > 0xFFFFFFu || raw.w > 0xFFFFFFu) bad = true;
+        if (id >= (1ull << 47) || e.src > 0xFFFFFFu || e.dest > 0xFFFFFFu) bad = true;
         uint32_t* o = reinterpret_cast<uint32_t*>(out) + (g - first) * 3;
         o[0] = (uint32_t)id;
-        o[1] = (uint32_t)((id >> 32) & 0x7FFFu) | (recv ? 0x8000u : 0u) | ((raw.z & 0xFFFFu) << 16);
-        o[2] = ((raw.z >> 16) & 0xFFu) | (raw.w << 8);
+        o[1] = (uint32_t)((id >> 32) & 0x7FFFu) | (recv ? 0x8000u : 0u) | ((e.src & 0xFFFFu) << 16);
+        o[2] = ((e.src >> 16) & 0xFFu) | (e.dest << 8);
       } else {
         uint4* o = reinterpret_cast<uint4*>(out) + (g - first) * 2;
-        event_rec(g, recv, tnow, id, raw, o[0], o[1]);
+        event_rec(g, tnow, e, o[0], o[1]);
       }
     }
   }
diff --git a/maelstrom_b200/engine.py b/maelstrom_b200/engine.py
--- a/maelstrom_b200/engine.py
+++ b/maelstrom_b200/engine.py
@@ -306,9 +306,10 @@
                 for i, cls in enumerate(("all", "clients", "servers"))}
 
     def counters(self):
-        out = np.zeros(8, dtype=np.uint64)
-        self._chk(self.L.ms_counters(self.h, out.ctypes.data))
-        names = ("rounds", "sends", "recvs", "launches", "lost", "partition_drops", "max_window", "fallback_sorts")
+        out = np.zeros(9, dtype=np.uint64)
+        self._chk(self.L.ms_counters_n(self.h, out.ctypes.data, out.size))
+        names = ("rounds", "sends", "recvs", "launches", "lost", "partition_drops", "max_window", "fallback_sorts",
+                 "wide_chunks")
         return {k: int(v) for k, v in zip(names, out)}
 
     RING_FIELDS = ("tail", "limit", "head", "ctail", "climit", "chead")
```
